# l13039968960/stm32H7-YOLO

Measured on AMD Instinct MI355X. Metric: images/sec int8 YOLO-face 56x56, higher is better.
Workload: dtype int8; 1 GPU; BASELINE configs[1]: batch=4096 int8 YOLO-face 56x56x3 frames per GPU, fused LDS-resident forward + GPU box decode; frames_per_gpu=4096, global_batch=4096, frame_bytes_in=9408, frame_bytes_out=882, input_batches_rotated=8, input_bytes_resident=308281344, kernel=yoloface56_fused<F=2,NW=8>, requant_rounding=ref, parallelism=single GPU, gather_every=1, collectives_issued=0, launch_streams=2

## Files before the change

stm32h7-yolo_amd/csrc/yf_decode.hip.h:

```cpp
#ifndef YF_DECODE_HIP_H
#define YF_DECODE_HIP_H
#include <hip/hip_runtime.h>
#include <stdint.h>
#include "../../include/yf_network.h"

namespace yfdec {

__device__ __constant__ uint32_t d_sig_bits[256];
__device__ __constant__ uint32_t d_exp_bits[256];

__device__ __forceinline__ int f2i_x86(float v) {
  return (v > -2147483904.0f && v < 2147483648.0f) ? (int)v : (int)0x80000000;
}
__device__ __forceinline__ int f2i_sat(float v) {
  return v != v ? 0 : (v >= 2147483648.0f ? 0x7FFFFFFF : (v <= -2147483648.0f ? (int)0x80000000 : (int)v));
}
__device__ __forceinline__ int dbl_wrap(int v) { return (int)((unsigned)v * 2u); }

__device__ __forceinline__ void decode_frame(const int8_t* head, long frame, int lane, int mode, float w_scale, float h_scale,
                                             yf_det* __restrict__ dets, int* __restrict__ counts, int cap) {
  yf_det* out = dets + frame * cap;
  const float anc_w[3] = {9.f, 12.f, 22.f}, anc_h[3] = {14.f, 17.f, 21.f};
  int total = 0;
  for (int base = 0; base < 147; base += 64) {
    const int i = base + lane;
    bool keep = false;
    int a = 0, row = 0, col = 0;
    const int8_t* p = head;
    float conf = 0.f;
    if (i < 147) {
      if (mode == YF_DECODE_PY) { a = i / 49; const int cell = i - a * 49; row = cell / 7; col = cell - row * 7; }
      else { const int cell = i / 3; a = i - cell * 3; row = cell / 7; col = cell - row * 7; }
      p = head + (row * 7 + col) * 18 + a * 6;
      conf = __uint_as_float(d_sig_bits[p[4] + 128]);
      keep = (mode == YF_DECODE_PY) ? (conf > 0.7f) : ((double)conf >= 0.7);
    }
    const unsigned long long mask = __ballot(keep);
    const int pos = total + __popcll(mask & ((1ull << lane) - 1ull));
    if (keep && pos < cap) {
      const float sx = __uint_as_float(d_sig_bits[p[0] + 128]), sy = __uint_as_float(d_sig_bits[p[1] + 128]);
      const float ew = __uint_as_float(d_exp_bits[p[2] + 128]), eh = __uint_as_float(d_exp_bits[p[3] + 128]);
      yf_det d;
      d.frame = (int32_t)frame; d.anchor = (uint8_t)a; d.row = (uint8_t)row; d.col = (uint8_t)col;
      d.q_conf = p[4]; d.conf = conf;
      const float cx = (sx + (float)col) * 8.f, cy = (sy + (float)row) * 8.f;
      const float bw = ew * anc_w[a], bh = eh * anc_h[a];
      if (mode == YF_DECODE_PY) {
        float x1 = cx - bw / 2, y1 = cy - bh / 2, x2 = cx + bw / 2, y2 = cy + bh / 2;
        x1 *= w_scale; x2 *= w_scale; y1 *= h_scale; y2 *= h_scale;
        d.x1 = f2i_x86(x1); d.y1 = f2i_x86(y1); d.x2 = f2i_x86(x2); d.y2 = f2i_x86(y2);
      } else {
        const float fy2 = cx - bw / 2, fy1 = cx + bw / 2, fx1 = cy - bh / 2, fx2 = cy + bh / 2;
        const bool arm = mode == YF_DECODE_FW;
        int y2 = arm ? f2i_sat(fy2) : f2i_x86(fy2), y1 = arm ? f2i_sat(fy1) : f2i_x86(fy1);
        int x1 = arm ? f2i_sat(fx1) : f2i_x86(fx1), x2 = arm ? f2i_sat(fx2) : f2i_x86(fx2);
        if (x1 < 0) x1 = 0;
        if (y1 < 0) y1 = 0;
        if (x2 > 55) x2 = 55;
        if (y2 > 55) y2 = 55;
        d.x1 = dbl_wrap(x1); d.y1 = dbl_wrap(y1); d.x2 = dbl_wrap(x2); d.y2 = dbl_wrap(y2);
      }
      out[pos] = d;
    }
    total += __popcll(mask);
  }
  if (lane == 0) counts[frame] = total;
}

typedef const __attribute__((address_space(3))) uint32_t* dec_lds_u32;
__device__ __forceinline__ void decode_frame_lds(const int8_t* head, long frame, int lane, int mode, float w_scale, float h_scale,
                                                 yf_det* __restrict__ dets, int* __restrict__ counts, int cap, uint32_t lds_tabs, int q_thr) {
  yf_det* out = dets + frame * cap;
  const float anc_w[3] = {9.f, 12.f, 22.f}, anc_h[3] = {14.f, 17.f, 21.f};
  auto sig = [&](int q) { return __uint_as_float(*(dec_lds_u32)(lds_tabs + 4u * (uint32_t)(q + 128))); };
  auto ex = [&](int q) { return __uint_as_float(*(dec_lds_u32)(lds_tabs + 1024u + 4u * (uint32_t)(q + 128))); };
  int pos[3], off[3], q4[3];
  bool keep[3];
  int total = 0;
#pragma unroll
  for (int c = 0; c < 3; ++c) {
    const int i = min(64 * c + lane, 146);
    if (mode == YF_DECODE_PY) { const int a = (i >= 49) + (i >= 98); off[c] = (i - 49 * a) * 18 + 6 * a; }
    else off[c] = 6 * i;
    q4[c] = head[off[c] + 4];
  }
#pragma unroll
  for (int c = 0; c < 3; ++c) {
    keep[c] = (64 * c + lane < 147) && q4[c] >= q_thr;
    const unsigned long long mask = __ballot(keep[c]);
    pos[c] = total + __popcll(mask & ((1ull << lane) - 1ull));
    total += __popcll(mask);
  }
#pragma unroll
  for (int c = 0; c < 3; ++c) {
    if (keep[c] && pos[c] < cap) {
      const int i = 64 * c + lane;
      int a, row, col;
      if (mode == YF_DECODE_PY) { a = i / 49; const int cell = i - a * 49; row = cell / 7; col = cell - row * 7; }
      else { const int cell = i / 3; a = i - cell * 3; row = cell / 7; col = cell - row * 7; }
      const int8_t* q = head + off[c];
      const float sx = sig(q[0]), sy = sig(q[1]), ew = ex(q[2]), eh = ex(q[3]);
      yf_det d;
      d.frame = (int32_t)frame; d.anchor = (uint8_t)a; d.row = (uint8_t)row; d.col = (uint8_t)col;
      d.q_conf = (int8_t)q4[c]; d.conf = sig(q4[c]);
      const float cx = (sx + (float)col) * 8.f, cy = (sy + (float)row) * 8.f;
      const float bw = ew * anc_w[a], bh = eh * anc_h[a];
      if (mode == YF_DECODE_PY) {
        float x1 = cx - bw / 2, y1 = cy - bh / 2, x2 = cx + bw / 2, y2 = cy + bh / 2;
        x1 *= w_scale; x2 *= w_scale; y1 *= h_scale; y2 *= h_scale;
        d.x1 = f2i_x86(x1); d.y1 = f2i_x86(y1); d.x2 = f2i_x86(x2); d.y2 = f2i_x86(y2);
      } else {
        const float fy2 = cx - bw / 2, fy1 = cx + bw / 2, fx1 = cy - bh / 2, fx2 = cy + bh / 2;
        const bool arm = mode == YF_DECODE_FW;
        int y2 = arm ? f2i_sat(fy2) : f2i_x86(fy2), y1 = arm ? f2i_sat(fy1) : f2i_x86(fy1);
        int x1 = arm ? f2i_sat(fx1) : f2i_x86(fx1), x2 = arm ? f2i_sat(fx2) : f2i_x86(fx2);
        if (x1 < 0) x1 = 0;
        if (y1 < 0) y1 = 0;
        if (x2 > 55) x2 = 55;
        if (y2 > 55) y2 = 55;
        d.x1 = dbl_wrap(x1); d.y1 = dbl_wrap(y1); d.x2 = dbl_wrap(x2); d.y2 = dbl_wrap(y2);
      }
      out[pos[c]] = d;
    }
  }
  if (lane == 0) counts[frame] = total;
}

}
#endif
```

stm32h7-yolo_amd/csrc/yf_engine.hip:

```cpp
#include <hip/hip_runtime.h>
#include <stdio.h>
#include <stdlib.h>
#include <string.h>
#include <condition_variable>
#include <deque>
#include <mutex>
#include <string>
#include <thread>
#include "yf_engine.h"
#include "yf_stream_scratch.h"
#include "yf_decode.hip.h"
#define YF_SET
#include "yf_kernel_set.hip.h"
#define YF_SET u
#define YF_RQ3_DENSE 1
#include "yf_kernel_set.hip.h"
#define YF_SET x
#define YF_RQ_FP32 1
#include "yf_kernel_set.hip.h"
#ifdef YF_LAB
#define YF_DUMP_PROD_ORDER 1
#define YF_SET
#include "yf_kernel_set.hip.h"
#define YF_SET u
#define YF_RQ3_DENSE 1
#include "yf_kernel_set.hip.h"
#undef YF_DUMP_PROD_ORDER
#endif
#include "gen/yf_decode_tables_gen.h"

namespace {

using yfdec::d_sig_bits;
using yfdec::d_exp_bits;

__global__ void __launch_bounds__(256) decode_kernel(const int8_t* __restrict__ heads, long n, int mode, float w_scale,
                                                     float h_scale, yf_det* __restrict__ dets, int* __restrict__ counts, int cap) {
  const int lane = threadIdx.x & 63;
  const long frame = (long)blockIdx.x * 4 + (threadIdx.x >> 6);
  if (frame >= n) return;
  yfdec::decode_frame(heads + frame * 882, frame, lane, mode, w_scale, h_scale, dets, counts, cap);
}

__global__ void __launch_bounds__(256) pack_dets_kernel(const yf_det* __restrict__ dets, const int* __restrict__ counts, const int8_t* __restrict__ heads,
                                                        uint32_t* __restrict__ wire, long n, int cap) {
  const long i = (long)blockIdx.x * 256 + threadIdx.x;
  if (i >= n * cap) return;
  const long f = i / cap;
  const int k = (int)(i - f * cap);
  uint32_t w0 = 0, w1 = 0, w2 = 0;
  if (k < min(counts[f], cap)) {
    const yf_det d = dets[i];
    const int8_t* q = heads + f * 882 + ((int)d.row * 7 + (int)d.col) * 18 + 6 * (int)d.anchor;
    w0 = (uint32_t)d.anchor | ((uint32_t)d.row << 8) | ((uint32_t)d.col << 16);
    w1 = (uint32_t)(uint8_t)q[0] | ((uint32_t)(uint8_t)q[1] << 8) | ((uint32_t)(uint8_t)q[2] << 16) | ((uint32_t)(uint8_t)q[3] << 24);
    w2 = (uint32_t)(uint8_t)q[4] | ((uint32_t)(uint8_t)q[5] << 8);
  }
  wire[3 * i] = w0; wire[3 * i + 1] = w1; wire[3 * i + 2] = w2;
}
__global__ void __launch_bounds__(256) unpack_dets_kernel(const uint32_t* __restrict__ wire, const int* __restrict__ counts, int8_t* __restrict__ heads, long n, int cap) {
  const int lane = threadIdx.x & 63;
  const long f = (long)blockIdx.x * 4 + (threadIdx.x >> 6);
  if (f >= n) return;
  int8_t* h = heads + f * 882;
  for (int b = lane; b < 882; b += 64) h[b] = (int8_t)-128;
  __builtin_amdgcn_wave_barrier();
  __threadfence_block();
  const int m = min(counts[f], cap);
  for (int k = lane; k < m; k += 64) {
    const uint32_t w0 = wire[3 * (f * cap + k)], w1 = wire[3 * (f * cap + k) + 1], w2 = wire[3 * (f * cap + k) + 2];
    const int a = (int)(w0 & 255u), row = (int)((w0 >> 8) & 255u), col = (int)((w0 >> 16) & 255u);
    if (a > 2 || row > 6 || col > 6) continue;
    int8_t* q = h + (row * 7 + col) * 18 + 6 * a;
    q[0] = (int8_t)(w1 & 255u); q[1] = (int8_t)((w1 >> 8) & 255u); q[2] = (int8_t)((w1 >> 16) & 255u); q[3] = (int8_t)(w1 >> 24);
    q[4] = (int8_t)(w2 & 255u); q[5] = (int8_t)((w2 >> 8) & 255u);
  }
}

__global__ void __launch_bounds__(256) prepare_rgb565_kernel(const uint8_t* __restrict__ src, int8_t* __restrict__ dst, long n) {
  const long i = (long)blockIdx.x * 256 + threadIdx.x;
  if (i >= n * 3136) return;
  const long f = i / 3136; const int r = (int)(i - f * 3136);
  const int y = r / 56, x = r - y * 56;
  const uint8_t* s = src + f * (112 * 112 * 2);
  unsigned sr = 0, sg = 0, sb = 0;
#pragma unroll
  for (int dy = 0; dy < 2; ++dy)
#pragma unroll
    for (int dx = 0; dx < 2; ++dx) {
      const int o = ((2 * y + dy) * 112 + (2 * x + dx)) * 2;
      const unsigned px = ((unsigned)s[o] << 8) | s[o + 1];
      sr += (px >> 11) & 0x1F; sg += (px >> 5) & 0x3F; sb += px & 0x1F;
    }
  const unsigned color = (((sr >> 2) & 0x1F) << 11) | (((sg >> 2) & 0x3F) << 5) | ((sb >> 2) & 0x1F);
  int8_t* o8 = dst + f * 9408 + r * 3;
  o8[0] = (int8_t)(((color & 0xF800) >> 8) - 128);
  o8[1] = (int8_t)(((color & 0x07E0) >> 3) - 128);
  o8[2] = (int8_t)(((color & 0x001F) << 3) - 128);
}

typedef void (*fused_fn)(const yf::NetParams);
enum Build { RUN, DUMP, DUMP_PROD_ORDER, CAMERA };
struct Variant { int f, nw, kset; Build build; fused_fn fn; size_t lds; size_t park; const char* name; };

#define YF_KERNEL_SETS(X) \
  X( , 0, "", "") \
  X(u, 1, ",sign-free dense epilogue", " (sign-free dense epilogue)") \
  X(x, 2, ",fp32 requantisation", " (fp32 requantisation)")
#define YF_VARIANT(NS, KSET, F, NW, BUILD, TAG) { F, NW, KSET, BUILD, (fused_fn)NS::yoloface56_fused<F, NW, BUILD == DUMP || BUILD == DUMP_PROD_ORDER, BUILD == CAMERA>, \
    NS::lds_bytes<F, NW, BUILD == DUMP || BUILD == DUMP_PROD_ORDER>(), NS::scratch_bytes_per_frame_slot<BUILD == DUMP || BUILD == DUMP_PROD_ORDER>(), \
    "yoloface56_fused<F=" #F ",NW=" #NW TAG ">" },
#define YF_PRODUCT_VARIANTS(S, KSET, LABEL, BAND_LABEL) \
  YF_VARIANT(yf##S, KSET, 2, 8, RUN, LABEL) YF_VARIANT(yf##S, KSET, 1, 8, RUN, LABEL) YF_VARIANT(yf##S, KSET, 2, 8, DUMP, LABEL) \
  YF_VARIANT(yf##S, KSET, 2, 8, CAMERA, ",RGB565 input" LABEL)
const Variant k_variants[] = {
  YF_KERNEL_SETS(YF_PRODUCT_VARIANTS)
#ifdef YF_LAB
  YF_VARIANT(yf, 0, 1, 4, RUN, "") YF_VARIANT(yf, 0, 2, 4, RUN, "") YF_VARIANT(yf, 0, 4, 8, RUN, "") YF_VARIANT(yf, 0, 2, 4, DUMP, "")
  YF_VARIANT(yfpd, 0, 2, 8, DUMP_PROD_ORDER, ",dump in production order")
  YF_VARIANT(yfpdu, 1, 2, 8, DUMP_PROD_ORDER, ",dump in production order,sign-free dense epilogue")
#endif
};

}

struct yf_engine {
  int device = 0;
  int cus = 0;
  size_t lds_per_cu = 0;
  int band_wgs_per_cu[3][3] = {{1, 1, 1}, {1, 1, 1}, {1, 1, 1}};
  int kset = 0;
#ifdef YF_LAB
  int grid_div = 1;
  int fail_next_launch = 0;
  bool dump_prod_order = false;
#endif
  uint8_t* d_tab = nullptr;
  yf_table_index ix;
  const Variant* var = nullptr;
  const Variant* var_dump = nullptr;
  void* d_in = nullptr; void* d_out = nullptr; long stage_cap = 0;
  bool layerwise160 = false;
  long chunk160 = 1024;
  yf_stream_scratch arena160;
  yf_stream_scratch park; size_t park_region = 0;
  hipStream_t own_stream = nullptr;
  hipEvent_t ev0 = nullptr, ev1 = nullptr;
  std::string err;
  uint32_t sig_bits[256], exp_bits[256];
  const Variant* var_small = nullptr;
  hipStream_t pipe_stream[2] = {nullptr, nullptr};
  hipEvent_t pipe_ev[2] = {nullptr, nullptr};
  void* h_small_in = nullptr; void* h_small_out = nullptr;
  struct Downloader* dl = nullptr;
};
constexpr long SMALL_N = 512;
constexpr long ZERO_COPY_N = 8;
constexpr long PIPE_MIN_N = 2048, PIPE_CHUNK_DEFAULT = 3072, PIPE_LAST_DEFAULT = 1024;

struct Downloader {
  struct Job { hipEvent_t ready; const void* src; void* dst; size_t bytes; };
  int device = 0;
  hipStream_t stream = nullptr;
  std::thread th;
  std::mutex mu;
  std::condition_variable cv_job, cv_idle;
  std::deque<Job> q;
  int pending = 0;
  bool stop = false;
  hipError_t status = hipSuccess;
  void loop() {
    (void)hipSetDevice(device);
    for (;;) {
      Job j;
      {
        std::unique_lock<std::mutex> lk(mu);
        cv_job.wait(lk, [&] { return stop || !q.empty(); });
        if (q.empty()) return;
        j = q.front(); q.pop_front();
      }
      hipError_t rc = hipStreamWaitEvent(stream, j.ready, 0);
      if (rc == hipSuccess) rc = hipMemcpyAsync(j.dst, j.src, j.bytes, hipMemcpyDeviceToHost, stream);
      if (rc == hipSuccess) rc = hipStreamSynchronize(stream);
      {
        std::lock_guard<std::mutex> lk(mu);
        if (rc != hipSuccess && status == hipSuccess) status = rc;
        --pending; cv_idle.notify_all();
      }
    }
  }
  hipError_t start(int dev) {
    device = dev;
    const hipError_t rc = hipStreamCreateWithFlags(&stream, hipStreamNonBlocking);
    if (rc != hipSuccess) return rc;
    th = std::thread([this] { loop(); });
    return hipSuccess;
  }
  void submit(const Job& j) { { std::lock_guard<std::mutex> lk(mu); q.push_back(j); ++pending; } cv_job.notify_one(); }
  hipError_t drain() { std::unique_lock<std::mutex> lk(mu); cv_idle.wait(lk, [&] { return pending == 0; }); const hipError_t rc = status; status = hipSuccess; return rc; }
  hipError_t drain_to(int below) { std::unique_lock<std::mutex> lk(mu); cv_idle.wait(lk, [&] { return pending < below; }); return status; }
  ~Downloader() {
    { std::lock_guard<std::mutex> lk(mu); stop = true; }
    cv_job.notify_all();
    if (th.joinable()) th.join();
    if (stream) (void)hipStreamDestroy(stream);
  }
};

#define HIPCHK(e_, call) do { hipError_t rc_ = (call); if (rc_ != hipSuccess) { \
    (e_)->err = std::string(#call) + ": " + hipGetErrorString(rc_); return YF_ENG_ERR_HIP; } } while (0)

static const Variant* shape_for(const yf_engine* e, long n);
static const Variant* find_variant(int f, int nw, int kset, Build build) {
  for (const Variant& v : k_variants) if (v.f == f && v.nw == nw && v.kset == kset && v.build == build) return &v;
  return nullptr;
}

static const Variant* dump_variant_for(const yf_engine* e, int f, int nw) {
#ifdef YF_LAB
  if (e->dump_prod_order) {
    const Variant* v = find_variant(f, nw, e->kset, DUMP_PROD_ORDER);
    if (v || e->kset == 2) return v;
  }
#endif
  return find_variant(f, nw, e->kset, DUMP);
}
static void select_variants(yf_engine* e, int f, int nw, bool automatic) {
  e->var = find_variant(f, nw, e->kset, RUN);
  e->var_dump = dump_variant_for(e, f, nw);
  e->var_small = automatic ? find_variant(1, 8, e->kset, RUN) : nullptr;
}

#ifdef YF_LAB
template <int ST>
static int launch160_from(yf_engine* e, const yf160::GenParams& prm, unsigned grid, hipStream_t s) {
  if constexpr (ST < yf160::GEN_STAGES) {
    hipLaunchKernelGGL((yf160::generic_stage_kernel<ST, 8>), dim3(grid), dim3(512), yf160::LUT_BYTES, s, prm);
    { hipError_t rc_ = hipGetLastError(); if (rc_ != hipSuccess) { e->err = std::string("generic stage launch: ") + hipGetErrorString(rc_); return YF_ENG_ERR_HIP; } }
    return launch160_from<ST + 1>(e, prm, grid, s);
  } else {
    return YF_ENG_OK;
  }
}

#endif

struct BandKernel { const void* fn; const char* name; unsigned threads; size_t lds; int jobs_per_frame; };
#ifndef YF_K1_NW
#define YF_K1_NW 8
#endif
#define YF_K1_NW_ YF_K1_NW
#define YF_BAND_KERNELS(S, KSET, LABEL, BAND_LABEL) \
  {{(const void*)yf160##S::band::band_k1<YF_K1_NW_>, "band_k1" BAND_LABEL, YF_K1_NW_ * 64, (size_t)yf160##S::band::K1_LDS, yf160##S::band::K1_BANDS}, \
   {(const void*)yf160##S::band::band_k23<8>, "band_k23" BAND_LABEL, 512, (size_t)yf160##S::band::K23_LDS, yf160##S::band::K23_BANDS}, \
   {(const void*)yf160##S::band::band_k4<8>,  "band_k4" BAND_LABEL, 512,  (size_t)yf160##S::band::K4_LDS, 1}},
static const BandKernel k_band_fused[3][3] = { YF_KERNEL_SETS(YF_BAND_KERNELS) };
static int launch160_banded(yf_engine* e, const yf160::band::Params& prm, hipStream_t s) {
  for (int i = 0; i < 3; ++i) {
    const BandKernel& k = k_band_fused[e->kset][i];
    const long jobs = prm.n * k.jobs_per_frame;
    const long full = (long)e->cus * e->band_wgs_per_cu[e->kset][i];
    const unsigned grid = (unsigned)(jobs < full ? jobs : full);
    void* args[] = {(void*)&prm};
    const hipError_t rc = hipLaunchKernel(k.fn, dim3(grid), dim3(k.threads), args, k.lds, s);
    if (rc != hipSuccess) { e->err = std::string(k.name) + " launch: " + hipGetErrorString(rc); return YF_ENG_ERR_HIP; }
  }
  return YF_ENG_OK;
}

static const char k_layout_refusal[] = "table blob layout differs from the layout compiled into the kernels";
static bool layout_is_the_compiled_plan(const yf_table_index* ix) {
  bool same = (int)ix->lut_off == yf::PLAN.lut_off && (int)ix->total_bytes == yf::PLAN.total;
  for (int i = 0; i < YF_N_DENSE; ++i) same = same && (int)ix->dense[i].w_off == yf::PLAN.w_off[i] && (int)ix->dense[i].c_off == yf::PLAN.c_off[i];
  for (int i = 0; i < YF_N_DW; ++i) same = same && (int)ix->dw[i].g_off == yf::PLAN.g_off[i];
  for (int i = 0; i < YF_N_CS; ++i)
    same = same && (int)ix->cs_v_off[i] == yf::PLAN.vb_off[i] && (int)ix->cs_v_bytes[i] == yf::PLAN.vb_bytes[i] && (int)ix->cs_s_off[i] == yf::PLAN.sb_off[i];
  return same;
}

template <typename Kernel, typename... Args>
static int launch_small(yf_engine* e, Kernel kernel, long threads, void* stream, Args... args) {
  if (threads == 0) return YF_ENG_OK;
  HIPCHK(e, hipSetDevice(e->device));
  hipLaunchKernelGGL(kernel, dim3((unsigned)((threads + 255) / 256)), dim3(256), 0, (hipStream_t)stream, args...);
  HIPCHK(e, hipGetLastError());
  return YF_ENG_OK;
}

static int upload_decode_tables(yf_engine* e, const uint32_t* sig, const uint32_t* ex) {
  for (int i = 1; i < 256; ++i) {
    float a, b; memcpy(&a, &sig[i - 1], 4); memcpy(&b, &sig[i], 4);
    if (!(b >= a)) { e->err = "sigmoid table is not monotonic"; return YF_ENG_ERR_ARG; }
  }
  HIPCHK(e, hipSetDevice(e->device));
  HIPCHK(e, hipDeviceSynchronize());
  HIPCHK(e, hipMemcpyToSymbol(HIP_SYMBOL(d_sig_bits), sig, 1024));
  HIPCHK(e, hipMemcpyToSymbol(HIP_SYMBOL(d_exp_bits), ex, 1024));
  memcpy(e->sig_bits, sig, 1024); memcpy(e->exp_bits, ex, 1024);
  return YF_ENG_OK;
}

extern "C" {

int yf_engine_set_decode_tables(yf_engine* e, const uint32_t* sig_bits, const uint32_t* exp_bits) {
  if (!e || !sig_bits || !exp_bits) return YF_ENG_ERR_ARG;
  return upload_decode_tables(e, sig_bits, exp_bits);
}
void yf_engine_get_decode_tables(const yf_engine* e, uint32_t* sig_bits, uint32_t* exp_bits) {
  memcpy(sig_bits, e->sig_bits, 1024); memcpy(exp_bits, e->exp_bits, 1024);
}

int yf_engine_create(int device, const uint8_t* table_blob, const yf_table_index* ix, int kernel_set, yf_engine** out, char* err, size_t errlen) {
  auto fail = [&](const std::string& m, int code) { if (err && errlen) snprintf(err, errlen, "%s", m.c_str()); return code; };
  if (!table_blob || !ix || !out) return fail("bad arguments", YF_ENG_ERR_ARG);
  int ndev = 0;
  hipError_t rc = hipGetDeviceCount(&ndev);
  if (rc != hipSuccess || ndev <= 0)
    return fail(std::string("no HIP device: ") + (rc != hipSuccess ? hipGetErrorString(rc) : "device count is 0"), YF_ENG_ERR_NO_DEVICE);
  if (device < 0 || device >= ndev) return fail("device index out of range", YF_ENG_ERR_ARG);
  yf_engine* e = new yf_engine();
  e->device = device; e->ix = *ix;
  e->arena160.max_regions = 4;
  auto bail = [&](hipError_t r, const char* what) { std::string m = std::string(what) + ": " + hipGetErrorString(r); yf_engine_destroy(e); return fail(m, YF_ENG_ERR_HIP); };
  auto quit = [&](const std::string& m, int code) { yf_engine_destroy(e); return fail(m, code); };
  if ((rc = hipSetDevice(device)) != hipSuccess) return bail(rc, "hipSetDevice");
  hipDeviceProp_t prop;
  if ((rc = hipGetDeviceProperties(&prop, device)) != hipSuccess) return bail(rc, "hipGetDeviceProperties");
  if (strncmp(prop.gcnArchName, "gfx950", 6) != 0) return quit(std::string("unsupported GPU ") + prop.gcnArchName + " (this library is gfx950 only)", YF_ENG_ERR_NO_DEVICE);
  e->cus = prop.multiProcessorCount;
  e->lds_per_cu = prop.maxSharedMemoryPerMultiProcessor;
  for (const Variant& v : k_variants)
    if (e->lds_per_cu < v.lds) return quit("the device reports " + std::to_string(e->lds_per_cu) + " bytes of LDS per CU, " + v.name + " needs " + std::to_string(v.lds), YF_ENG_ERR_NO_DEVICE);
  if (!layout_is_the_compiled_plan(ix)) return quit(k_layout_refusal, YF_ENG_ERR_ARG);
  if ((rc = hipMalloc((void**)&e->d_tab, ix->total_bytes)) != hipSuccess) return bail(rc, "hipMalloc(tables)");
  if ((rc = hipMemcpy(e->d_tab, table_blob, ix->total_bytes, hipMemcpyHostToDevice)) != hipSuccess) return bail(rc, "hipMemcpy(tables)");
  if (upload_decode_tables(e, yf_sigmoid_bits, yf_exp_bits) != YF_ENG_OK) { const std::string m = e->err; return quit(m, YF_ENG_ERR_HIP); }
  auto prepare_kernel = [&](const void* fn, const std::string& refusal, size_t lds, unsigned threads = 0, int* wgs_per_cu = nullptr) -> int {
    hipFuncAttributes at;
    if ((rc = hipFuncGetAttributes(&at, fn)) != hipSuccess) return bail(rc, "hipFuncGetAttributes");
    if (at.sharedSizeBytes != 0) return quit(refusal, YF_ENG_ERR_HIP);
    if (lds && (rc = hipFuncSetAttribute(fn, hipFuncAttributeMaxDynamicSharedMemorySize, (int)lds)) != hipSuccess) return bail(rc, "hipFuncSetAttribute(max dynamic LDS)");
    if (!wgs_per_cu) return YF_ENG_OK;
    int occ = 0;
    if ((rc = hipOccupancyMaxActiveBlocksPerMultiprocessor(&occ, fn, (int)threads, lds)) != hipSuccess) return bail(rc, "hipOccupancyMaxActiveBlocksPerMultiprocessor");
    *wgs_per_cu = occ > 0 ? occ : 1;
    return YF_ENG_OK;
  };
  const std::string static_lds = ": kernel has static LDS, absolute LUT addressing is invalid";
  int r;
  for (const Variant& v : k_variants) if ((r = prepare_kernel((const void*)v.fn, v.name + static_lds, v.lds)) != YF_ENG_OK) return r;
#ifdef YF_LAB
  if ((r = prepare_kernel((const void*)yf160::generic_stage_kernel<1, 8>, "generic stage kernel has static LDS", 0)) != YF_ENG_OK) return r;
  { const char* lw = getenv("YF_160_LAYERWISE"); e->layerwise160 = lw && lw[0] == '1'; }
#endif
  for (int u = 0; u < 3; ++u)
    for (int i = 0; i < 3; ++i) {
      const BandKernel& k = k_band_fused[u][i];
      if ((r = prepare_kernel(k.fn, k.name + static_lds, k.lds, k.threads, &e->band_wgs_per_cu[u][i])) != YF_ENG_OK) return r;
    }
  { const char* ck = getenv("YF_160_CHUNK"); if (ck && atol(ck) > 0) e->chunk160 = atol(ck); }
#ifdef YF_LAB
  { const char* fl = getenv("YF_LAB_FAIL_LAUNCHES"); if (fl) e->fail_next_launch = atoi(fl); }
  { const char* gd = getenv("YF_LAB_GRID_DIV"); if (gd && atoi(gd) > 1) e->grid_div = atoi(gd); }
  { const char* pd = getenv("YF_LAB_DUMP_PROD_ORDER"); e->dump_prod_order = pd && pd[0] == '1'; }
#endif
  {
    size_t park = 0;
    for (const Variant& v : k_variants) park = v.park > park ? v.park : park;
    size_t slots = 4;
    for (const Variant& v : k_variants) { const size_t need = (e->lds_per_cu / v.lds) * (size_t)v.f; slots = need > slots ? need : slots; }
    e->park_region = (size_t)e->cus * slots * park;
  }
  if ((rc = hipStreamCreate(&e->own_stream)) != hipSuccess) return bail(rc, "hipStreamCreate");
  if ((rc = hipEventCreate(&e->ev0)) != hipSuccess || (rc = hipEventCreate(&e->ev1)) != hipSuccess) return bail(rc, "hipEventCreate");
  for (int k = 0; k < 2; ++k) {
    if ((rc = hipStreamCreateWithFlags(&e->pipe_stream[k], hipStreamNonBlocking)) != hipSuccess) return bail(rc, "hipStreamCreateWithFlags");
    if ((rc = hipEventCreateWithFlags(&e->pipe_ev[k], hipEventDisableTiming)) != hipSuccess) return bail(rc, "hipEventCreateWithFlags");
  }
  if ((rc = hipHostMalloc(&e->h_small_in, (size_t)ZERO_COPY_N * 9408, hipHostMallocMapped)) != hipSuccess ||
      (rc = hipHostMalloc(&e->h_small_out, (size_t)ZERO_COPY_N * 882, hipHostMallocMapped)) != hipSuccess) return bail(rc, "hipHostMalloc(pinned staging)");
  e->kset = kernel_set;
  select_variants(e, 2, 8, true);
  *out = e;
  return YF_ENG_OK;
}

int yf_engine_set_tables(yf_engine* e, const uint8_t* table_blob, const yf_table_index* ix, int kernel_set) {
  if (!e || !table_blob || !ix) return YF_ENG_ERR_ARG;
  if (!find_variant(e->var->f, e->var->nw, kernel_set, RUN)) { e->err = "the configured kernel shape has no build for this rounding"; return YF_ENG_ERR_VARIANT; }
  if (!layout_is_the_compiled_plan(ix)) { e->err = k_layout_refusal; return YF_ENG_ERR_ARG; }
  HIPCHK(e, hipSetDevice(e->device));
  HIPCHK(e, hipDeviceSynchronize());
  HIPCHK(e, hipMemcpy(e->d_tab, table_blob, ix->total_bytes, hipMemcpyHostToDevice));
  e->ix = *ix;
  const bool automatic = e->var_small != nullptr;
  e->kset = kernel_set;
  select_variants(e, e->var->f, e->var->nw, automatic);
  return YF_ENG_OK;
}

void yf_engine_destroy(yf_engine* e) {
  if (!e) return;
  (void)hipSetDevice(e->device);
  (void)hipDeviceSynchronize();
  if (e->d_tab) (void)hipFree(e->d_tab);
  if (e->d_in) (void)hipFree(e->d_in);
  if (e->d_out) (void)hipFree(e->d_out);
  e->arena160.release();
  e->park.release();
  if (e->ev0) (void)hipEventDestroy(e->ev0);
  if (e->ev1) (void)hipEventDestroy(e->ev1);
  if (e->own_stream) (void)hipStreamDestroy(e->own_stream);
  delete e->dl;
  for (int k = 0; k < 2; ++k) {
    if (e->pipe_ev[k]) (void)hipEventDestroy(e->pipe_ev[k]);
    if (e->pipe_stream[k]) (void)hipStreamDestroy(e->pipe_stream[k]);
  }
  if (e->h_small_in) (void)hipHostFree(e->h_small_in);
  if (e->h_small_out) (void)hipHostFree(e->h_small_out);
  delete e;
}

int yf_engine_table_plan(int32_t* out, int cap) {
  const int need = 2 * YF_N_DENSE + YF_N_DW + 2 + 3 * YF_N_CS;
  if (!out || cap < need) return need;
  int k = 0;
  for (int i = 0; i < YF_N_DENSE; ++i) out[k++] = yf::PLAN.w_off[i];
  for (int i = 0; i < YF_N_DENSE; ++i) out[k++] = yf::PLAN.c_off[i];
  for (int i = 0; i < YF_N_DW; ++i) out[k++] = yf::PLAN.g_off[i];
  out[k++] = yf::PLAN.lut_off; out[k++] = yf::PLAN.total;
  for (int i = 0; i < YF_N_CS; ++i) out[k++] = yf::PLAN.vb_off[i];
  for (int i = 0; i < YF_N_CS; ++i) out[k++] = yf::PLAN.vb_bytes[i];
  for (int i = 0; i < YF_N_CS; ++i) out[k++] = yf::PLAN.sb_off[i];
  return need;
}

int yf_engine_variant_exists(int frames_per_wg, int waves_per_wg) { return find_variant(frames_per_wg, waves_per_wg, 0, RUN) != nullptr; }

int yf_engine_configure(yf_engine* e, int frames_per_wg, int waves_per_wg) {
  if (!e) return YF_ENG_ERR_ARG;
  if (frames_per_wg < 0) {
    select_variants(e, 2, 8, true);
    return YF_ENG_OK;
  }
  const int f = frames_per_wg > 0 ? frames_per_wg : e->var->f, nw = waves_per_wg > 0 ? waves_per_wg : e->var->nw;
  if (!find_variant(f, nw, e->kset, RUN)) { e->err = "no such kernel variant"; return YF_ENG_ERR_VARIANT; }
  select_variants(e, f, nw, false);
  return YF_ENG_OK;
}

const char* yf_engine_error(const yf_engine* e) { return e ? e->err.c_str() : "null engine"; }
const char* yf_engine_kernel_name(const yf_engine* e) { return e && e->var ? e->var->name : ""; }
const char* yf_engine_kernel_name_for(const yf_engine* e, long n) { return e && e->var ? shape_for(e, n)->name : ""; }
#ifndef YF_BUILD_ID
#define YF_BUILD_ID "unstamped"
#endif
const char* yf_engine_build_id(void) { return YF_BUILD_ID; }
long yf_engine_dump_bytes(void) { return yf::DumpOffsets::TOTAL; }

static int yf_decode_q_threshold(const yf_engine* e, int mode) {
  for (int i = 0; i < 256; ++i) {
    float v; memcpy(&v, &e->sig_bits[i], 4);
    if (mode == YF_DECODE_PY ? (v > 0.7f) : ((double)v >= 0.7)) return i - 128;
  }
  return 128;
}
static bool decode_mode_ok(int mode) { return mode == YF_DECODE_PY || mode == YF_DECODE_FW || mode == YF_DECODE_FW_HOST; }
struct DecodeArgs { void* dets; void* counts; int cap, mode; float w_scale, h_scale; };

static const Variant* shape_for(const yf_engine* e, long n) { return (e->var_small && n <= SMALL_N) ? e->var_small : e->var; }

static int launch(yf_engine* e, const Variant* v, const void* d_in, void* d_out, void* d_dump, long n, hipStream_t s, int stop_stage = -1,
                  const DecodeArgs* dec = nullptr) {
  if (n <= 0) return YF_ENG_OK;
  if (((uintptr_t)d_in & 3) != 0) { e->err = "input must be 4-byte aligned"; return YF_ENG_ERR_ARG; }
  if (((uintptr_t)d_out & 1) != 0) { e->err = "output must be 2-byte aligned"; return YF_ENG_ERR_ARG; }
  yf::NetParams prm;
  prm.in = (const int8_t*)d_in; prm.out = (int8_t*)d_out; prm.n = n; prm.tab = e->d_tab; prm.dump = (int8_t*)d_dump; prm.stop_stage = stop_stage;
  prm.dets = nullptr; prm.counts = nullptr; prm.cap = 0; prm.mode = 0; prm.w_scale = prm.h_scale = 1.f;
  prm.q_thr = 128;
  if (dec) { prm.dets = (yf_det*)dec->dets; prm.counts = (int*)dec->counts; prm.cap = dec->cap; prm.mode = dec->mode; prm.w_scale = dec->w_scale; prm.h_scale = dec->h_scale;
             prm.q_thr = yf_decode_q_threshold(e, dec->mode); }
  const long groups = (n + v->f - 1) / v->f;
  const int per_cu = (int)(e->lds_per_cu / v->lds) > 0 ? (int)(e->lds_per_cu / v->lds) : 1;
  long grid = (long)e->cus * per_cu;
#ifdef YF_LAB
  if (e->grid_div > 1) grid = grid / e->grid_div > 0 ? grid / e->grid_div : 1;
#endif
  if (grid > groups) grid = groups;
  prm.scratch = nullptr;
  yf_stream_scratch::Lease lease;
  if (v->park) {
    const size_t need = (size_t)grid * v->f * v->park;
    if (need > e->park_region) { e->err = "tail scratch region too small for this kernel shape"; return YF_ENG_ERR_VARIANT; }
    HIPCHK(e, e->park.get(s, e->park_region, &lease));
    prm.scratch = lease.ptr;
  }
#ifdef YF_LAB
  if (e->fail_next_launch > 0) { --e->fail_next_launch; grid = 0; }
#endif
  hipLaunchKernelGGL(v->fn, dim3((unsigned)grid), dim3(v->nw * 64), v->lds, s, prm);
  HIPCHK(e, hipGetLastError());
  HIPCHK(e, lease.mark());
  return YF_ENG_OK;
}

int yf_engine_run_device(yf_engine* e, const void* d_in, void* d_out, void* d_dump, long n, void* stream) {
  if (!e || !d_in || !d_out || n < 0) return YF_ENG_ERR_ARG;
  HIPCHK(e, hipSetDevice(e->device));
#ifdef YF_BARPROF
  return launch(e, e->var, d_in, d_out, d_dump, n, (hipStream_t)stream);
#else
  if (d_dump && !e->var_dump) { e->err = "no debug (dump) build of the configured kernel shape"; return YF_ENG_ERR_VARIANT; }
  return launch(e, d_dump ? e->var_dump : shape_for(e, n), d_in, d_out, d_dump, n, (hipStream_t)stream);
#endif
}

int yf_engine_run_decode_device(yf_engine* e, const void* d_in, void* d_out, long n, int mode, float w_scale, float h_scale,
                                void* d_dets, void* d_counts, int cap, void* stream) {
  if (!e || !d_in || !d_out || !d_dets || !d_counts || n < 0 || cap <= 0 || !decode_mode_ok(mode)) return YF_ENG_ERR_ARG;
  HIPCHK(e, hipSetDevice(e->device));
  const DecodeArgs dec = {d_dets, d_counts, cap, mode, w_scale, h_scale};
  return launch(e, shape_for(e, n), d_in, d_out, nullptr, n, (hipStream_t)stream, -1, &dec);
}

int yf_engine_run_camera_device(yf_engine* e, const void* d_rgb565, void* d_out, long n, int mode, float w_scale, float h_scale,
                                void* d_dets, void* d_counts, int cap, void* stream) {
  if (!e || !d_rgb565 || !d_out || n < 0) return YF_ENG_ERR_ARG;
  if (d_dets && (!d_counts || cap <= 0 || !decode_mode_ok(mode))) return YF_ENG_ERR_ARG;
  if (((uintptr_t)d_rgb565 & 15) != 0) { e->err = "camera frames must be 16-byte aligned"; return YF_ENG_ERR_ARG; }
  HIPCHK(e, hipSetDevice(e->device));
  const Variant* v = find_variant(e->var->f, e->var->nw, e->kset, CAMERA);
  if (!v) { e->err = "no camera-input build of the configured kernel shape"; return YF_ENG_ERR_VARIANT; }
  const DecodeArgs dec = {d_dets, d_counts, cap, mode, w_scale, h_scale};
  return launch(e, v, d_rgb565, d_out, nullptr, n, (hipStream_t)stream, -1, d_dets ? &dec : nullptr);
}

int yf_engine_run_host(yf_engine* e, const void* h_in, void* h_out, long n) {
  if (!e || !h_in || n < 0) return YF_ENG_ERR_ARG;
  if (n == 0) return YF_ENG_OK;
  HIPCHK(e, hipSetDevice(e->device));
  if (n <= ZERO_COPY_N) {
    memcpy(e->h_small_in, h_in, (size_t)n * 9408);
    void *d_i = nullptr, *d_o = nullptr;
    HIPCHK(e, hipHostGetDevicePointer(&d_i, e->h_small_in, 0));
    HIPCHK(e, hipHostGetDevicePointer(&d_o, e->h_small_out, 0));
    const int rc = launch(e, shape_for(e, n), d_i, d_o, nullptr, n, e->own_stream);
    if (rc) return rc;
    HIPCHK(e, hipStreamSynchronize(e->own_stream));
    if (h_out) memcpy(h_out, e->h_small_out, (size_t)n * 882);
    return YF_ENG_OK;
  }
  if (n > e->stage_cap) {
    if (e->d_in) (void)hipFree(e->d_in);
    if (e->d_out) (void)hipFree(e->d_out);
    e->d_in = e->d_out = nullptr; e->stage_cap = 0;
    HIPCHK(e, hipMalloc(&e->d_in, (size_t)n * 9408));
    HIPCHK(e, hipMalloc(&e->d_out, (size_t)n * 882));
    e->stage_cap = n;
  }
  if (n < PIPE_MIN_N) {
    HIPCHK(e, hipMemcpyAsync(e->d_in, h_in, (size_t)n * 9408, hipMemcpyHostToDevice, e->own_stream));
    const int rc = launch(e, shape_for(e, n), e->d_in, e->d_out, nullptr, n, e->own_stream);
    if (rc) return rc;
    if (h_out) HIPCHK(e, hipMemcpyAsync(h_out, e->d_out, (size_t)n * 882, hipMemcpyDeviceToHost, e->own_stream));
    HIPCHK(e, hipStreamSynchronize(e->own_stream));
    return YF_ENG_OK;
  }
  if (h_out && !e->dl) {
    e->dl = new Downloader();
    const hipError_t rc = e->dl->start(e->device);
    if (rc != hipSuccess) { delete e->dl; e->dl = nullptr; e->err = std::string("download stream: ") + hipGetErrorString(rc); return YF_ENG_ERR_HIP; }
  }
  static const long PIPE_CHUNK = [] { const char* v = getenv("YF_PIPE_CHUNK"); const long c = v ? atol(v) : 0; return c >= 256 ? c : PIPE_CHUNK_DEFAULT; }();
  static const long PIPE_LAST = [] { const char* v = getenv("YF_PIPE_LAST"); const long c = v ? atol(v) : 0; return c >= 64 ? c : PIPE_LAST_DEFAULT; }();
  int rc = YF_ENG_OK;
  hipError_t hrc = hipSuccess;
  long done = 0;
  for (int k = 0; done < n && rc == YF_ENG_OK && hrc == hipSuccess; ++k) {
    long c = n - done < PIPE_CHUNK ? n - done : PIPE_CHUNK;
    if (c == n - done && c > 2 * PIPE_LAST) c -= PIPE_LAST;
    hipStream_t st = e->pipe_stream[k & 1];
    const char* src = (const char*)h_in + done * 9408;
    char* d_i = (char*)e->d_in + done * 9408;
    char* d_o = (char*)e->d_out + done * 882;
    if (h_out && k >= 2) { const hipError_t r = e->dl->drain_to(2); if (r != hipSuccess) { hrc = r; break; } }
    hrc = hipMemcpyAsync(d_i, src, (size_t)c * 9408, hipMemcpyHostToDevice, st);
    if (hrc != hipSuccess) break;
    rc = launch(e, e->var, d_i, d_o, nullptr, c, st);
    if (rc != YF_ENG_OK) break;
    if (h_out) {
      hrc = hipEventRecord(e->pipe_ev[k & 1], st);
      if (hrc != hipSuccess) break;
      e->dl->submit(Downloader::Job{e->pipe_ev[k & 1], d_o, (char*)h_out + done * 882, (size_t)c * 882});
    }
    done += c;
  }
  const hipError_t d_rc = e->dl && h_out ? e->dl->drain() : hipSuccess;
  const hipError_t s0 = hipStreamSynchronize(e->pipe_stream[0]), s1 = hipStreamSynchronize(e->pipe_stream[1]);
  if (rc != YF_ENG_OK) return rc;
  for (hipError_t r : {hrc, d_rc, s0, s1}) if (r != hipSuccess) { e->err = std::string("pipelined host run: ") + hipGetErrorString(r); return YF_ENG_ERR_HIP; }
  return YF_ENG_OK;
}

int yf_engine_run_host_dump(yf_engine* e, const void* h_in, void* h_out, void* h_dump, long n) {
  if (!e || !h_in || !h_out || !h_dump || n <= 0) return YF_ENG_ERR_ARG;
  if (!e->var_dump) { e->err = "no debug (dump) build of the configured kernel shape"; return YF_ENG_ERR_VARIANT; }
  HIPCHK(e, hipSetDevice(e->device));
  const size_t ds = (size_t)yf::DumpOffsets::TOTAL;
  char *d_i = nullptr, *d_o = nullptr, *d_d = nullptr;
  int rc = YF_ENG_OK;
  hipError_t h = hipMalloc((void**)&d_i, (size_t)n * 9408);
  if (h == hipSuccess) h = hipMalloc((void**)&d_o, (size_t)n * 882);
  if (h == hipSuccess) h = hipMalloc((void**)&d_d, (size_t)n * ds);
  if (h == hipSuccess) h = hipMemcpyAsync(d_i, h_in, (size_t)n * 9408, hipMemcpyHostToDevice, e->own_stream);
  if (h == hipSuccess) rc = launch(e, e->var_dump, d_i, d_o, d_d, n, e->own_stream);
  if (h == hipSuccess && rc == YF_ENG_OK) h = hipMemcpyAsync(h_out, d_o, (size_t)n * 882, hipMemcpyDeviceToHost, e->own_stream);
  if (h == hipSuccess && rc == YF_ENG_OK) h = hipMemcpyAsync(h_dump, d_d, (size_t)n * ds, hipMemcpyDeviceToHost, e->own_stream);
  const hipError_t hs = hipStreamSynchronize(e->own_stream);
  if (d_i) (void)hipFree(d_i);
  if (d_o) (void)hipFree(d_o);
  if (d_d) (void)hipFree(d_d);
  if (rc != YF_ENG_OK) return rc;
  if (h != hipSuccess || hs != hipSuccess) { e->err = std::string("observed run: ") + hipGetErrorString(h != hipSuccess ? h : hs); return YF_ENG_ERR_HIP; }
  return YF_ENG_OK;
}

long yf_engine_dump_offset(int tflite_op) {
  typedef yf::DumpOffsets D;
  switch (tflite_op) {
    case 2: return D::T1; case 4: return D::T2; case 5: return D::T3; case 7: return D::T4; case 21: return D::Q21; case 11: return D::T6;
    case 12: return D::T7; case 14: return D::T8; case 16: return D::T9; case 18: return D::T11; case 22: return D::T14; case 24: return D::T15;
    case 45: return D::Q45; case 28: return D::T17; case 29: return D::T18; case 31: return D::T19; case 33: return D::T20; case 35: return D::T22;
    case 37: return D::T23; case 39: return D::T24; case 41: return D::T26; case 46: return D::T30; case 48: return D::T31; case 50: return D::T32;
    case 52: return D::T33; case 8: return D::P8; case 17: return D::C17; case 25: return D::P25; case 34: return D::C34; case 40: return D::C40;
    case 43: return D::L43;
    default: return -1;
  }
}

static int time_launches(yf_engine* e, const Variant* v, const void* d_in, void* d_out, long n, int iters, int stop_stage, void* stream, float* ms_per_launch) {
  HIPCHK(e, hipSetDevice(e->device));
  hipStream_t s = (hipStream_t)stream;
  HIPCHK(e, hipEventRecord(e->ev0, s));
  for (int i = 0; i < iters; ++i) { const int rc = launch(e, v, d_in, d_out, nullptr, n, s, stop_stage); if (rc) return rc; }
  HIPCHK(e, hipEventRecord(e->ev1, s));
  HIPCHK(e, hipEventSynchronize(e->ev1));
  float ms = 0.f;
  HIPCHK(e, hipEventElapsedTime(&ms, e->ev0, e->ev1));
  *ms_per_launch = ms / iters;
  return YF_ENG_OK;
}

int yf_engine_time_device(yf_engine* e, const void* d_in, void* d_out, long n, int iters, void* stream, float* ms_per_launch) {
  if (!e || !d_in || !d_out || n <= 0 || iters <= 0 || !ms_per_launch) return YF_ENG_ERR_ARG;
  return time_launches(e, e->var, d_in, d_out, n, iters, -1, stream, ms_per_launch);
}

int yf_engine_time_stages(yf_engine* e, const void* d_in, void* d_out, long n, int iters, int stop_stage, void* stream, float* ms_per_launch) {
  if (!e || !d_in || !d_out || n <= 0 || iters <= 0 || !ms_per_launch) return YF_ENG_ERR_ARG;
  if (!e->var_dump) { e->err = "no debug (stage-timing) build of the configured kernel shape"; return YF_ENG_ERR_VARIANT; }
  return time_launches(e, e->var_dump, d_in, d_out, n, iters, stop_stage, stream, ms_per_launch);
}

int yf_engine_run_device_160(yf_engine* e, const void* d_in, void* d_out, long n, void* stream) {
  if (!e || !d_in || !d_out || n < 0) return YF_ENG_ERR_ARG;
  if (n == 0) return YF_ENG_OK;
  if (((uintptr_t)d_in & 3) != 0 || ((uintptr_t)d_out & 1) != 0) { e->err = "input must be 4-byte, output 2-byte aligned"; return YF_ENG_ERR_ARG; }
  HIPCHK(e, hipSetDevice(e->device));
  const long cap = n < e->chunk160 ? n : e->chunk160;
#ifdef YF_LAB
  const size_t per_frame = e->layerwise160 ? (size_t)yf160::FRAME_BYTES : (size_t)yf160::band::ARENA_BYTES;
#else
  const size_t per_frame = (size_t)yf160::band::ARENA_BYTES;
#endif
  yf_stream_scratch::Lease lease;
  HIPCHK(e, e->arena160.get((hipStream_t)stream, (size_t)cap * per_frame, &lease));
  char* arena = lease.ptr;
  for (long done = 0; done < n; done += cap) {
    const long m = (n - done) < cap ? (n - done) : cap;
    int rc;
#ifdef YF_LAB
    if (e->layerwise160) {
      if (e->kset == 2) { e->err = "the layer-by-layer 160x160 form has no float32-requantisation build (YF_160_LAYERWISE with YF_ROUND_FP32)"; return YF_ENG_ERR_VARIANT; }
      yf160::GenParams prm;
      prm.in = (const int8_t*)d_in + done * yf160::IN_FRAME_BYTES;
      prm.out = (int8_t*)d_out + done * yf160::OUT_FRAME_BYTES;
      prm.n = m; prm.tab = e->d_tab; prm.arena = arena;
      rc = launch160_from<0>(e, prm, (unsigned)m, (hipStream_t)stream);
    } else
#endif
    {
      yf160::band::Params prm;
      prm.in = (const int8_t*)d_in + done * yf160::IN_FRAME_BYTES;
      prm.out = (int8_t*)d_out + done * yf160::OUT_FRAME_BYTES;
      prm.n = m; prm.tab = e->d_tab; prm.arena = arena;
      rc = launch160_banded(e, prm, (hipStream_t)stream);
    }
    if (rc) return rc;
  }
  HIPCHK(e, lease.mark());
  return YF_ENG_OK;
}

int yf_engine_release_stream(yf_engine* e, void* stream) {
  if (!e) return YF_ENG_ERR_ARG;
  HIPCHK(e, hipSetDevice(e->device));
  HIPCHK(e, e->park.release_stream((hipStream_t)stream));
  HIPCHK(e, e->arena160.release_stream((hipStream_t)stream));
  return YF_ENG_OK;
}

size_t yf_engine_scratch_bytes(yf_engine* e) { return e ? e->park.bytes_held() + e->arena160.bytes_held() : 0; }
void yf_engine_scratch_stats(yf_engine* e, unsigned long long out[6]) {
  for (int i = 0; i < 6; ++i) out[i] = 0;
  if (!e) return;
  for (yf_stream_scratch* m : {&e->park, &e->arena160}) {
    const yf_stream_scratch::Stats s = m->stats();
    out[0] += s.events_recorded; out[1] += s.events_skipped; out[2] += s.event_waits; out[3] += s.device_syncs; out[4] += s.acquire_waits; out[5] += s.regions;
  }
}

int yf_engine_decode_device(yf_engine* e, const void* d_heads, long n, int mode, float w_scale, float h_scale,
                            void* d_dets, void* d_counts, int cap, void* stream) {
  if (!e || !d_heads || !d_dets || !d_counts || n < 0 || cap <= 0 || !decode_mode_ok(mode)) return YF_ENG_ERR_ARG;
  return launch_small(e, decode_kernel, n * 64, stream, (const int8_t*)d_heads, n, mode, w_scale, h_scale, (yf_det*)d_dets, (int*)d_counts, cap);
}

int yf_engine_pack_detections_device(yf_engine* e, const void* d_dets, const void* d_counts, const void* d_heads, void* d_wire, long n, int cap, void* stream) {
  if (!e || !d_dets || !d_counts || !d_heads || !d_wire || n < 0 || cap <= 0 || ((uintptr_t)d_wire & 3) != 0 || ((uintptr_t)d_dets & 3) != 0) return YF_ENG_ERR_ARG;
  return launch_small(e, pack_dets_kernel, n * cap, stream, (const yf_det*)d_dets, (const int*)d_counts, (const int8_t*)d_heads, (uint32_t*)d_wire, n, cap);
}

int yf_engine_unpack_detections_device(yf_engine* e, const void* d_wire, const void* d_counts, void* d_heads, long n, int cap, void* stream) {
  if (!e || !d_wire || !d_counts || !d_heads || n < 0 || cap <= 0 || ((uintptr_t)d_wire & 3) != 0) return YF_ENG_ERR_ARG;
  return launch_small(e, unpack_dets_kernel, n * 64, stream, (const uint32_t*)d_wire, (const int*)d_counts, (int8_t*)d_heads, n, cap);
}

int yf_engine_prepare_rgb565_device(yf_engine* e, const void* d_rgb565, void* d_out, long n, void* stream) {
  if (!e || !d_rgb565 || !d_out || n < 0) return YF_ENG_ERR_ARG;
  return launch_small(e, prepare_rgb565_kernel, n * 3136, stream, (const uint8_t*)d_rgb565, (int8_t*)d_out, n);
}

}
```

stm32h7-yolo_amd/csrc/yf_fused56.hip.h:

```cpp


template <class B, int C, int F, int NT>
__device__ __forceinline__ void dump_buf(const char* frames, int8_t* dump, long stride, long off, long first_frame,
                                         long n_frames, int tid, int ch0 = 0, int split = 1 << 30, int gap = 0) {
  if (!dump) return;
  for (int i = tid; i < F * B::P * C; i += NT) {
    const int ch = i % C; const int t = i / C;
    const int p = t % B::P; const int f = t / B::P;
    if (first_frame + f >= n_frames) continue;
    const int phys = ch0 + ch + (ch >= split ? gap : 0);
    dump[(first_frame + f) * stride + off + (long)p * C + ch] = (int8_t)frames[f * B::FS + B::at_p(p) + phys];
  }
}

template <class B, int C, int FT, int NT, class IdOf>
__device__ __forceinline__ void dump_sets(const char* frames, int8_t* dump, long stride, long off, const IdOf& id_of, int tid, int ch0 = 0, int split = 1 << 30, int gap = 0) {
  for (int i = tid; i < FT * B::P * C; i += NT) {
    const int ch = i % C; const int t = i / C;
    const int p = t % B::P; const int f = t / B::P;
    const long id = id_of(f);
    if (id < 0) continue;
    const int phys = ch0 + ch + (ch >= split ? gap : 0);
    dump[id * stride + off + (long)p * C + ch] = (int8_t)frames[f * B::FS + B::at_p(p) + phys];
  }
}

struct DumpOffsets {
  enum { T1 = 0, T2 = T1 + 6272, T3 = T2 + 6272, T4 = T3 + 3136, Q21 = T4 + 14112, T6 = Q21 + 3528, T7 = T6 + 3528,
         T8 = T7 + 1176, T9 = T8 + 7056, T11 = T9 + 7056, T14 = T11 + 1176, T15 = T14 + 7056, Q45 = T15 + 4704,
         T17 = Q45 + 1176, T18 = T17 + 1176, T19 = T18 + 392, T20 = T19 + 1960, T22 = T20 + 1960, T23 = T22 + 392,
         T24 = T23 + 1960, T26 = T24 + 1960, T30 = T26 + 392, T31 = T30 + 2352, T32 = T31 + 1960, T33 = T32 + 1960,
         P8 = T33 + 1568, C17 = P8 + 3528, P25 = C17 + 1176, C34 = P25 + 1176, C40 = C34 + 392, L43 = C40 + 392,
         TOTAL = L43 + 1176 };
};

struct NetParams {
  const int8_t* in;
  int8_t* out;
  long n;
  const uint8_t* tab;
  int8_t* dump;
  int stop_stage;
  yf_det* dets;
  int* counts;
  int cap, mode;
  int q_thr;
  float w_scale, h_scale;
  char* scratch;
};
static_assert(sizeof(yf_table_index) <= YF_INDEX_RESERVED, "index does not fit its reserved slot");

#ifndef YF_POOL_MERGE
#define YF_POOL_MERGE 1
#endif
#ifndef YF_POOL8H_WAVES
#define YF_POOL8H_WAVES 3
#endif
#ifndef YF_POOL8V_WAVES
#define YF_POOL8V_WAVES 3
#endif
#ifndef YF_PRIO_LIST
#define YF_PRIO_LIST 3,3,3,3,3,3,3,3,3,3, 2,2,2,2, 1,1,1,1,1,1, 0,0,0,0,0,0,0
#endif
constexpr int STAGE_PRIO[27] = {YF_PRIO_LIST};
template <int K> __device__ __forceinline__ void stage_prio() {
  if constexpr (K == 0 || STAGE_PRIO[K] != STAGE_PRIO[K - 1]) __builtin_amdgcn_s_setprio(STAGE_PRIO[K]);
}
#if defined(YF_LAB) && defined(YF_DUMP_PROD_ORDER)
#define YF_PDUMP 1
#else
#define YF_PDUMP 0
#endif
template <bool DUMP> constexpr bool tail_batch() { return !DUMP || YF_PDUMP; }

template <int F, int NW, bool DUMP, bool CAM = false>
#if !defined(YF_LAB) || !defined(YF_TPJ13)
#undef YF_TPJ13
#define YF_TPJ13 3
#endif
#if !defined(YF_LAB) || !defined(YF_TPJ23)
#undef YF_TPJ23
#define YF_TPJ23 2
#endif
#if defined(YF_LAB) && defined(YF_WHATIF_WPE)
#define YF_WPE(NW) YF_WHATIF_WPE
#else
#define YF_WPE(NW) ((NW) == 12 ? 6 : (NW) >= 8 ? 4 : ((NW) == 6 ? 3 : 2))
#endif
__global__ void __launch_bounds__(NW * 64, YF_WPE(NW)) yoloface56_fused(const NetParams prm) {
  extern __shared__ __attribute__((aligned(16))) char smem[];
  constexpr int NT = NW * 64;
  constexpr bool BATCH = tail_batch<DUMP>();
  constexpr bool POOL_MERGE = YF_POOL_MERGE != 0 && (!DUMP || YF_PDUMP) && NW >= 8;
  constexpr bool XDUMP = DUMP && !YF_PDUMP;
  typedef Buf<B_T14::OFF, 14, 14, 32, 14, 0, 0> B_T6X;
  typedef typename std::conditional<POOL_MERGE, B_T6X, B_T6>::type B_T6M;
  constexpr int FT = BATCH ? 2 * F : F;
  typedef TailBufs<BATCH ? FRAME_STRIDE / 2 : FRAME_STRIDE> U;
  constexpr int OUT_ALL_BYTES = BATCH ? 0 : (F * OUT_FRAME_BYTES + 15) & ~15;
  uint8_t* luts = reinterpret_cast<uint8_t*>(smem);
  constexpr int PRE = v2::pre_bytes<F, tail_batch<DUMP>()>();
  char* out_all = smem + PRE;
  char* frames = smem + PRE + OUT_ALL_BYTES;
  long parked_first = -1;
  const int tid0 = threadIdx.x;
  const uint8_t* __restrict__ tab = prm.tab;
  int vz = 0;
  asm volatile("" : "+v"(vz));
  for (int i = tid0; i < v2::LUT_B / 16; i += NT)
    reinterpret_cast<uint4*>(luts)[i] = reinterpret_cast<const uint4*>(tab + PLAN.lut_off)[i];
  for (int i = tid0; i < v2::ZERO_B / 16; i += NT) reinterpret_cast<uint4*>(smem + v2::ZERO)[i] = uint4{0, 0, 0, 0};
  constexpr int DBG_LUT = PRE + OUT_ALL_BYTES + FRAME_BYTES + (F - 1) * FRAME_STRIDE;
  if constexpr (DUMP) { if (tid0 < YF_DBG_LUT_BYTES / 16) reinterpret_cast<uint4*>(smem + DBG_LUT)[tid0] = reinterpret_cast<const uint4*>(tab + PLAN.lut_off + YF_N_LUT * 256 + YF_ADDLUT_BYTES)[tid0]; }
#if !(defined(YF_LAB) && defined(YF_WHATIF_NO_PROLOGUE_TABLES))
  {
    typedef v2::JobTabs<F, tail_batch<DUMP>()> JTS;
    typedef typename JTS::U UT;
    v2::fill_jobtab<F, 1, B_T1, B_T2, JTS::JT_DW3>(smem, tid0);
    v2::fill_jobtab<F, 2, B_T4, B_T6M, JTS::JT_DW10>(smem, tid0);
    v2::fill_jobtab<F, 1, B_T8, B_T9, JTS::JT_DW15>(smem, tid0);
    v2::fill_jobtab<JTS::FT, 2, typename UT::T15, typename UT::T17, JTS::JT_DW27>(smem, tid0);
    v2::fill_jobtab<JTS::FT, 1, typename UT::T19, typename UT::T20, JTS::JT_DW32>(smem, tid0);
    typedef v2::HaloTabs<F, tail_batch<DUMP>()> HTS;
    v2::build_halotab<typename HTS::G1, HTS::H_T1, NT>(smem, tid0);
    v2::build_halotab<typename HTS::G4, HTS::H_T4, NT>(smem, tid0);
    v2::build_halotab<typename HTS::G8, HTS::H_T8, NT>(smem, tid0);
    v2::build_halotab<typename HTS::G15, HTS::H_T15, NT>(smem, tid0);
    v2::build_halotab<typename HTS::G19, HTS::H_T19, NT>(smem, tid0);
  }
#endif

  const long n_groups = (prm.n + F - 1) / F;
  const AddK no_add = {};
  auto addctx = [&](int k) {
    const uint8_t* a = tab + offsetof(yf_table_index, add) + k * sizeof(yf_add);
    return AddK{uniform_u32(a + offsetof(yf_add, mo2)), uniform_u32(a + offsetof(yf_add, zro)),
                (unsigned long)uniform_u32(a + offsetof(yf_add, c64o)) | ((unsigned long)uniform_u32(a + offsetof(yf_add, c64o) + 4) << 32),
                (int)uniform_u32(a + offsetof(yf_add, rso))};
  };
  constexpr long DS = DumpOffsets::TOTAL;
#ifdef YF_BARPROF
  bool prof_on = false;
  int bar_no = 0;
  long long* prof_out = reinterpret_cast<long long*>(prm.dump) + ((long)blockIdx.x * NW + __builtin_amdgcn_readfirstlane(tid0 >> 6)) * 80;
#define YF_SYNC() do { asm volatile("s_waitcnt vmcnt(0)" ::: "memory");    \
                       if (prof_on && (tid0 & 63) == 0 && bar_no < 40) prof_out[2 * bar_no] = __builtin_readcyclecounter(); __syncthreads(); \
                       if (prof_on && (tid0 & 63) == 0 && bar_no < 40) prof_out[2 * bar_no + 1] = __builtin_readcyclecounter(); ++bar_no; } while (0)
#else
#define YF_SYNC() do { asm volatile("s_waitcnt vmcnt(0)" ::: "memory"); __syncthreads(); } while (0)
#endif
#define YF_HALO(B, RING, FR, G, HOFF, WI, TID) \
  v2::fill_halo_t<B, typename v2::HaloTabs<F, BATCH>::G, v2::HaloTabs<F, BATCH>::HOFF>(frames, load_halo_zp(tab, WI), TID)
#define YF_FETCH(CS, WV, LN) v2::fetch_consts<CS>(tab, WV, LN)
#define YF_CONV1(WV, LN, CS) v2::conv1_2_stage<F, NW, CS>(frames, tab, WV, LN)
#define YF_DENSE(FR, TPJ, KS, BW, IN, OUT, CH0, COUT, EPI, LUT, ADDB, DI, AD, WV, LN, CS) \
  v2::dense2_stage<FR, NW, TPJ, KS, BW, IN, OUT, CH0, COUT, EPI, LUT, ADDB, CS>(frames, out_all, tab, AD, WV, LN)
#define YF_DW(FR, STRIDE, IN, OUT, C, LUT, WI, WV, LN, CS, JTOFF) v2::dw2_stage<FR, NW, STRIDE, IN, OUT, C, LUT, CS, v2::JobTabs<F, BATCH>::JTOFF>(frames, tab, WV, LN)
#define YF_DUMP(BUF, C, OFF, ...) \
  if constexpr (DUMP) { if (prm.dump) { dump_buf<BUF, C, F, NT>(frames, prm.dump, DS, DumpOffsets::OFF, first, prm.n, tid, ##__VA_ARGS__); YF_SYNC(); } }
  int stage_no = 0;
#define YF_STAGE_END() if constexpr (DUMP) { if (++stage_no == prm.stop_stage) continue; }
#define YF_PRIO(K) stage_prio<K>()

  long prev_first = -1;
  auto decode_prev = [&](int w, int ln) {
    if (prm.dets != nullptr && prev_first >= 0 && w >= NW - F && prev_first + (w - (NW - F)) < prm.n) {
      int dl = ln;
      asm volatile("" : "+v"(dl));
      yfdec::decode_frame(reinterpret_cast<const int8_t*>(out_all) + (w - (NW - F)) * OUT_FRAME_BYTES, prev_first + (w - (NW - F)), dl,
                          prm.mode, prm.w_scale, prm.h_scale, prm.dets, prm.counts, prm.cap);
    }
  };
  for (long grp = blockIdx.x; grp < n_groups; grp += gridDim.x) {
    const long first = grp * F;
#ifdef YF_BARPROF
    bar_no = 0;
    prof_on = !DUMP && prm.dump != nullptr && grp == (long)blockIdx.x + gridDim.x;
#endif
    int tid = tid0, tid_f = tid0, tid_m = tid0, tid_t = tid0;
    if constexpr ((YF_LAUNDER & 1) != 0) asm volatile("" : "+v"(tid_f));
    if constexpr ((YF_LAUNDER & 2) != 0) asm volatile("" : "+v"(tid_m));
    if constexpr ((YF_LAUNDER & 4) != 0) asm volatile("" : "+v"(tid_t));
    const int lane = tid & 63;
    const int wave = __builtin_amdgcn_readfirstlane(tid >> 6);
    const int L_f = tid_f & 63, L_m = tid_m & 63, L_t = tid_t & 63;
    const int W_f = __builtin_amdgcn_readfirstlane(tid_f >> 6), W_m = __builtin_amdgcn_readfirstlane(tid_m >> 6), W_t = __builtin_amdgcn_readfirstlane(tid_t >> 6);
    (void)lane; (void)wave;
#if !defined(YF_BARPROF)
    asm volatile("s_waitcnt lgkmcnt(0)\n\ts_barrier" ::: "memory");
#else
    YF_SYNC();
#endif
    stage_no = 0;
    YF_PRIO(0);
    int tid_s = tid0;
    asm volatile("" : "+v"(tid_s));
    if constexpr (CAM) stage_input_cam<F, NT>(frames, reinterpret_cast<const uint8_t*>(prm.in), first, prm.n, (int)uniform_u32(tab + offsetof(yf_table_index, in_zp)), tid_s);
    else stage_input<F, NT>(frames, prm.in, first, prm.n, (int)uniform_u32(tab + offsetof(yf_table_index, in_zp)), tid_s);
    YF_FETCH(0, W_f, L_f);
    YF_HALO(B_T1, true, F, G1, H_T1, YF_W_DW3, tid_f);
    YF_SYNC();
    YF_STAGE_END()
    YF_PRIO(1);
    YF_FETCH(1, W_f, L_f);
    YF_CONV1(W_f, L_f, 0);
    YF_SYNC(); YF_DUMP(B_T1, 8, T1)
    YF_STAGE_END()
    YF_PRIO(2);
    YF_FETCH(2, W_f, L_f);
    YF_DW(F, 1, B_T1, B_T2, 8, YF_L_LEAKY4, YF_W_DW3, W_f, L_f, 1, JT_DW3);
    YF_SYNC(); YF_DUMP(B_T2, 8, T2)
    YF_STAGE_END()
    YF_PRIO(3);
    YF_FETCH(3, W_f, L_f);
    YF_DENSE(F, 1, 1, 8, B_T2, B_T3, 0, 4, EPI_RAW, 0, B_T3, YF_D_C5, no_add, W_f, L_f, 2);
    YF_SYNC(); YF_DUMP(B_T3, 4, T3)
    YF_STAGE_END()
    YF_PRIO(4);
    YF_HALO(B_T4, false, F, G4, H_T4, YF_W_DW10, tid_f);
    YF_FETCH(4, W_f, L_f);
    YF_DENSE(F, 5, 1, 4, B_T3, B_T4, 0, 18, EPI_LUT, YF_L_LEAKY7, B_T4, YF_D_C6, no_add, W_f, L_f, 3);
    YF_SYNC(); YF_DUMP(B_T4, 18, T4)
    YF_STAGE_END()
    if constexpr (POOL_MERGE) {
      constexpr int PH = YF_POOL8H_WAVES, PV = YF_POOL8V_WAVES;
      YF_PRIO(5);
      YF_FETCH(5, W_m, L_m);
      if (W_m < PH) pool8_h<F, PH * 64>(frames, tid_m);
      else v2::dw2_stage<F, NW - PH, 2, B_T4, B_T6M, 18, YF_L_LEAKY11, 4, v2::JobTabs<F, BATCH>::JT_DW10>(frames, tab, W_m - PH, L_m);
      YF_SYNC(); YF_DUMP(B_T6M, 18, T6)
      YF_PRIO(8);
      YF_FETCH(6, W_m, L_m);
      YF_DENSE(F, 1, 2, 16, B_T6M, B_T7, 0, 6, EPI_RAW, 0, B_T7, YF_D_C12, no_add, W_m, L_m, 5);
      YF_SYNC(); YF_DUMP(B_T7, 6, T7)
      YF_PRIO(9);
      YF_HALO(B_T8, true, F, G8, H_T8, YF_W_DW15, tid_m);
      YF_FETCH(7, W_m, L_m);
      if (W_m < PV) pool8_v<F, PV * 64, false>(frames, tid_m);
      else v2::dense2_stage<F, NW - PV, YF_TPJ13, 1, 8, B_T7, B_T8, 0, 36, EPI_LUT, YF_L_LEAKY14, B_T8, 6>(frames, out_all, tab, no_add, W_m - PV, L_m);
      YF_SYNC(); YF_DUMP(B_T14, 18, Q21) YF_DUMP(B_T8, 36, T8)
    } else {
  YF_PRIO(5);
#if !(defined(YF_LAB) && defined(YF_WHATIF_NO_POOL8H))
      pool8_h<F, NT>(frames, tid_f);
      YF_SYNC();
#endif
      YF_STAGE_END()
      YF_PRIO(6);
      pool8_v<F, NT, XDUMP>(frames, tid_m);
      YF_SYNC();
      YF_PRIO(7);
      YF_FETCH(5, W_m, L_m);
      YF_DW(F, 2, B_T4, B_T6, 18, YF_L_LEAKY11, YF_W_DW10, W_m, L_m, 4, JT_DW10);
      YF_SYNC(); YF_DUMP(B_T14, 18, Q21) YF_DUMP(B_T14, 18, P8, YF_T14_CONV_BASE) YF_DUMP(B_T6, 18, T6)
      YF_STAGE_END()
      YF_PRIO(8);
      YF_FETCH(6, W_m, L_m);
      YF_DENSE(F, 1, 2, 16, B_T6, B_T7, 0, 6, EPI_RAW, 0, B_T7, YF_D_C12, no_add, W_m, L_m, 5);
      YF_SYNC(); YF_DUMP(B_T7, 6, T7)
      YF_STAGE_END()
      YF_PRIO(9);
      YF_HALO(B_T8, true, F, G8, H_T8, YF_W_DW15, tid_m);
      YF_FETCH(7, W_m, L_m);
      YF_DENSE(F, YF_TPJ13, 1, 8, B_T7, B_T8, 0, 36, EPI_LUT, YF_L_LEAKY14, B_T8, YF_D_C13, no_add, W_m, L_m, 6);
      YF_SYNC(); YF_DUMP(B_T8, 36, T8)
      YF_STAGE_END()
    }
    YF_PRIO(10);
    YF_FETCH(8, W_m, L_m);
    YF_DW(F, 1, B_T8, B_T9, 36, YF_L_LEAKY16, YF_W_DW15, W_m, L_m, 7, JT_DW15);
    YF_SYNC(); YF_DUMP(B_T9, 36, T9)
    YF_STAGE_END()
    YF_PRIO(11);
    YF_FETCH(9, W_m, L_m);
    if constexpr (XDUMP)
      v2::dense2_stage<F, NW, 1, 3, 16, B_T9, B_T11, 0, 6, EPI_ADD, YF_A_ADD18, B_T7, 8, B_T14::OFF + YF_T14_CONV_BASE, B_T14::S>(frames, out_all, tab, addctx(YF_A_ADD18), W_m, L_m);
    else
    YF_DENSE(F, 1, 3, 16, B_T9, B_T11, 0, 6, EPI_ADD, YF_A_ADD18, B_T7, YF_D_C17, addctx(YF_A_ADD18), W_m, L_m, 8);
    YF_SYNC(); YF_DUMP(B_T11, 6, T11) if constexpr (XDUMP) { YF_DUMP(B_T14, 6, C17, YF_T14_CONV_BASE) }
    YF_STAGE_END()
    YF_PRIO(12);
    YF_FETCH(10, W_m, L_m);
    YF_DENSE(F, 3, 1, 8, B_T11, B_T14, YF_T14_CONV_BASE, 18, EPI_LUT, YF_L_LEAKY20, B_T14, YF_D_C19, no_add, W_m, L_m, 9);
    YF_SYNC(); YF_DUMP(B_T14, 36, T14, 0, 18, 2)
    YF_STAGE_END()
    YF_PRIO(13);
    if constexpr (BATCH) {
      if (parked_first >= 0) {
        constexpr int PV = TailBufs<FRAME_BYTES>::T15_BYTES / 16, WI = (PV + 63) / 64;
        const char* park = prm.scratch + (long)blockIdx.x * (F * PV * 16);
        for (int j = W_m; j < F * WI; j += NW) {
          const int f = j / WI, k0 = (j - f * WI) * 64;
          if (k0 + L_m < PV)
            __builtin_amdgcn_global_load_lds((const __attribute__((address_space(1))) void*)(uintptr_t)(park + (f * PV + k0 + L_m) * 16),
                                             (__attribute__((address_space(3))) void*)(uintptr_t)(uint32_t)(PRE + (2 * f + 1) * U::T15::FS + 16 * k0),
                                             16, 0, 0);
        }
      }
    }
    YF_HALO(B_T15, false, F, G15, H_T15, YF_W_DW27, tid_m);
    YF_FETCH(11, W_m, L_m);
    YF_DENSE(F, YF_TPJ23, 3, 16, B_T14, B_T15, 0, 24, EPI_LUT, YF_L_LEAKY24, B_T15, YF_D_C23, no_add, W_m, L_m, 10);
    if constexpr (BATCH) asm volatile("s_waitcnt vmcnt(0)" ::: "memory");
    YF_SYNC(); YF_DUMP(B_T15, 24, T15)
    YF_STAGE_END()
    long odd_first = -1;
    if constexpr (BATCH) {
      constexpr int V = U::T15_BYTES / 16;
      uint4* park = reinterpret_cast<uint4*>(prm.scratch) + (long)blockIdx.x * (F * V);
      if (parked_first < 0 && grp + gridDim.x < n_groups) {
        for (int i = tid_t; i < F * V; i += NT) {
          const int f = i / V, k = i - f * V;
          park[i] = *reinterpret_cast<const uint4*>(frames + f * FRAME_STRIDE + 16 * k);
        }
        parked_first = first;
        continue;
      }
      if (parked_first >= 0) {
        odd_first = parked_first;
        parked_first = -1;
      }
    }
    auto frame_of = [&](int f) -> long {
      long id = first + f;
      if constexpr (BATCH) id = (f & 1) ? (odd_first >= 0 ? odd_first + (f >> 1) : -1) : first + (f >> 1);
      return id < prm.n ? id : -1;
    };
#define YF_DUMP_T(BUF, C, OFF, ...) \
  if constexpr (DUMP) { if (prm.dump) { if constexpr (BATCH) dump_sets<BUF, C, FT, NT>(frames, prm.dump, DS, DumpOffsets::OFF, frame_of, tid, ##__VA_ARGS__); \
                                        else dump_buf<BUF, C, FT, NT>(frames, prm.dump, DS, DumpOffsets::OFF, first, prm.n, tid, ##__VA_ARGS__); \
                                        YF_SYNC(); } }
    YF_PRIO(14);
    YF_FETCH(12, W_t, L_t);
    {
      constexpr int PW = v2::pool25_waves<FT>();
      static_assert(PW < NW, "waves left for conv2d_27");
      if (W_t < PW) v2::pool25_cols<FT, typename U::T15, typename U::T30, XDUMP>(frames, W_t * 64 + L_t);
      else v2::dw2_stage<FT, NW - PW, 2, typename U::T15, typename U::T17, 24, YF_L_LEAKY28, 11, v2::JobTabs<F, BATCH>::JT_DW27>(frames, tab, W_t - PW, L_t);
    }
    YF_SYNC(); YF_DUMP_T(typename U::T30, 24, Q45) if constexpr (XDUMP) { YF_DUMP_T(typename U::T30, 24, P25, 24) } YF_DUMP_T(typename U::T17, 24, T17)
    YF_STAGE_END()
    YF_PRIO(15);
    YF_FETCH(13, W_t, L_t);
    YF_DENSE(FT, 1, 2, 16, typename U::T17, typename U::T18, 0, 8, EPI_RAW, 0, typename U::T18, YF_D_C29, no_add, W_t, L_t, 12);
    if constexpr (!BATCH) decode_prev(W_t, L_t);
    YF_SYNC(); YF_DUMP_T(typename U::T18, 8, T18)
    YF_STAGE_END()
    YF_PRIO(16);
    YF_HALO(typename U::T19, true, FT, G19, H_T19, YF_W_DW32, tid_t);
    YF_FETCH(14, W_t, L_t);
    YF_DENSE(FT, 5, 1, 8, typename U::T18, typename U::T19, 0, 40, EPI_LUT, YF_L_LEAKY31, typename U::T19, YF_D_C30, no_add, W_t, L_t, 13);
    YF_SYNC(); YF_DUMP_T(typename U::T19, 40, T19)
    YF_STAGE_END()
    YF_PRIO(17);
    YF_FETCH(15, W_t, L_t);
    YF_DW(FT, 1, typename U::T19, typename U::T20, 40, YF_L_LEAKY33, YF_W_DW32, W_t, L_t, 14, JT_DW32);
    YF_SYNC(); YF_DUMP_T(typename U::T20, 40, T20)
    YF_STAGE_END()
    YF_PRIO(18);
    YF_FETCH(16, W_t, L_t);
    if constexpr (XDUMP)
      v2::dense2_stage<FT, NW, 1, 3, 16, typename U::T20, typename U::T22, 0, 8, EPI_ADD, YF_A_ADD35, typename U::T18, 15, U::T30::OFF + 24, U::T30::S>(frames, out_all, tab, addctx(YF_A_ADD35), W_t, L_t);
    else
    YF_DENSE(FT, 1, 3, 16, typename U::T20, typename U::T22, 0, 8, EPI_ADD, YF_A_ADD35, typename U::T18, YF_D_C34, addctx(YF_A_ADD35), W_t, L_t, 15);
    YF_SYNC(); YF_DUMP_T(typename U::T22, 8, T22) if constexpr (XDUMP) { YF_DUMP_T(typename U::T30, 8, C34, 24) }
    YF_STAGE_END()
    YF_PRIO(19);
    YF_HALO(typename U::T19, true, FT, G19, H_T19, YF_W_DW38, tid_t);
    YF_FETCH(17, W_t, L_t);
    YF_DENSE(FT, 5, 1, 8, typename U::T22, typename U::T19, 0, 40, EPI_LUT, YF_L_LEAKY37, typename U::T19, YF_D_C36, no_add, W_t, L_t, 16);
    YF_SYNC(); YF_DUMP_T(typename U::T19, 40, T23)
    YF_STAGE_END()
    YF_PRIO(20);
    YF_FETCH(18, W_t, L_t);
    YF_DW(FT, 1, typename U::T19, typename U::T20, 40, YF_L_LEAKY39, YF_W_DW38, W_t, L_t, 17, JT_DW32);
    YF_SYNC(); YF_DUMP_T(typename U::T20, 40, T24)
    YF_STAGE_END()
    YF_PRIO(21);
    YF_FETCH(19, W_t, L_t);
    if constexpr (XDUMP)
      v2::dense2_stage<FT, NW, 1, 3, 16, typename U::T20, typename U::T26, 0, 8, EPI_ADD, YF_A_ADD41, typename U::T22, 18, U::T30::OFF + 24, U::T30::S>(frames, out_all, tab, addctx(YF_A_ADD41), W_t, L_t);
    else
    YF_DENSE(FT, 1, 3, 16, typename U::T20, typename U::T26, 0, 8, EPI_ADD, YF_A_ADD41, typename U::T22, YF_D_C40, addctx(YF_A_ADD41), W_t, L_t, 18);
    YF_SYNC(); YF_DUMP_T(typename U::T26, 8, T26) if constexpr (XDUMP) { YF_DUMP_T(typename U::T30, 8, C40, 24) }
    YF_STAGE_END()
    YF_PRIO(22);
    YF_FETCH(20, W_t, L_t);
    if constexpr (XDUMP)
      v2::dense2_stage<FT, NW, 2, 1, 8, typename U::T26, typename U::T30, 24, 24, EPI_LUT, YF_L_L43Q44, typename U::T30, 19, U::T20::OFF, U::T20::S, DBG_LUT>(frames, out_all, tab, no_add, W_t, L_t);
    else
    YF_DENSE(FT, 3, 1, 8, typename U::T26, typename U::T30, 24, 24, EPI_LUT, YF_L_L43Q44, typename U::T30, YF_D_C42, no_add, W_t, L_t, 19);
    YF_SYNC(); YF_DUMP_T(typename U::T30, 48, T30) if constexpr (XDUMP) { YF_DUMP_T(typename U::T20, 24, L43) }
    YF_STAGE_END()
    YF_PRIO(23);
    YF_HALO(typename U::T19, true, FT, G19, H_T19, YF_W_DW49, tid_t);
    YF_FETCH(21, W_t, L_t);
    YF_DENSE(FT, 2, 3, 16, typename U::T30, typename U::T19, 0, 40, EPI_LUT, YF_L_LEAKY48, typename U::T19, YF_D_C47, no_add, W_t, L_t, 20);
    YF_SYNC(); YF_DUMP_T(typename U::T19, 40, T31)
    YF_STAGE_END()
    YF_PRIO(24);
    YF_FETCH(22, W_t, L_t);
    YF_DW(FT, 1, typename U::T19, typename U::T20, 40, YF_L_LEAKY50, YF_W_DW49, W_t, L_t, 21, JT_DW32);
    YF_SYNC(); YF_DUMP_T(typename U::T20, 40, T32)
    YF_STAGE_END()
    YF_PRIO(25);
    YF_FETCH(23, W_t, L_t);
    if (BATCH && prm.dets != nullptr && W_t < 2) {
      int dl = L_t;
      asm volatile("" : "+v"(dl));
      const uint8_t* src = reinterpret_cast<const uint8_t*>(W_t == 0 ? yfdec::d_sig_bits : yfdec::d_exp_bits) + 16 * dl;
      const uint32_t dst = (uint32_t)(PRE + OUT_ALL_BYTES + 1024 * W_t);
      uint32_t keep;
      asm volatile("s_mov_b32 %0, m0\n\ts_mov_b32 m0, %2\n\ts_nop 0\n\tglobal_load_lds_dwordx4 %1, off\n\ts_mov_b32 m0, %0"
                   : "=&s"(keep) : "v"(src), "s"(dst) : "memory");
    }
    YF_DENSE(FT, 2, 3, 16, typename U::T20, typename U::T33, 0, 32, EPI_LUT, YF_L_LEAKY52, typename U::T33, YF_D_C51, no_add, W_t, L_t, 22);
    YF_SYNC(); YF_DUMP_T(typename U::T33, 32, T33)
    YF_STAGE_END()
    YF_PRIO(26);
    if constexpr (!BATCH) {
      YF_DENSE(FT, 1, 2, 16, typename U::T33, typename U::T33, 0, 18, EPI_HEAD, 0, typename U::T33, YF_D_C53, no_add, W_t, L_t, 23);
      YF_SYNC();
      const long valid = min((long)F, prm.n - first);
      const int n16 = (int)(valid * (OUT_FRAME_BYTES / 2));
      uint16_t* dst = reinterpret_cast<uint16_t*>(prm.out + first * OUT_FRAME_BYTES);
      const uint16_t* srcp = reinterpret_cast<const uint16_t*>(out_all);
      for (int i = tid; i < n16; i += NT) dst[i] = srcp[i];
      prev_first = first;
    } else {
      YF_DENSE(FT, 1, 2, 16, typename U::T33, typename U::HEAD, 0, 18, EPI_HEAD_LDS, 0, typename U::T33, YF_D_C53, no_add, W_t, L_t, 23);
      YF_SYNC();
      constexpr int H16 = OUT_FRAME_BYTES / 2;
      const bool split = prm.dets != nullptr && FT < NW;
      const int c0 = split ? tid_t - FT * 64 : tid_t, cstep = split ? NT - FT * 64 : NT;
      if (!split || W_t >= FT) {
        for (int i = c0; i < FT * H16; i += cstep) {
          const int f = i / H16, k = i - f * H16;
          const long id = frame_of(f);
          if (id >= 0) reinterpret_cast<uint16_t*>(prm.out + id * OUT_FRAME_BYTES)[k] = *reinterpret_cast<const uint16_t*>(frames + f * U::HEAD::FS + U::HEAD::OFF + 2 * k);
        }
      }
      for (int f = W_t; f < FT; f += NW) {
        const long id = frame_of(f);
        if (prm.dets != nullptr && id >= 0) {
          int dl = L_t;
          asm volatile("" : "+v"(dl));
          yfdec::decode_frame_lds(reinterpret_cast<const int8_t*>(frames + f * U::HEAD::FS + U::HEAD::OFF), id, dl, prm.mode, prm.w_scale, prm.h_scale, prm.dets, prm.counts, prm.cap,
                                  (uint32_t)(PRE + OUT_ALL_BYTES), prm.q_thr);
        }
      }
    }
#undef YF_DUMP_T
  }
  if constexpr (!BATCH) {
    const int tid = tid0, lane = tid & 63, wave = __builtin_amdgcn_readfirstlane(tid >> 6);
    decode_prev(wave, lane);
  }
#undef YF_HALO
#undef YF_FETCH
#undef YF_CONV1
#undef YF_DENSE
#undef YF_DW
#undef YF_DUMP
#undef YF_STAGE_END
#undef YF_PRIO
#undef YF_SYNC
}

template <int F, int NW, bool DUMP>
constexpr size_t lds_bytes() { return (size_t)v2::pre_bytes<F, tail_batch<DUMP>()>() + (tail_batch<DUMP>() ? 0 : (F * OUT_FRAME_BYTES + 15) & ~15) + (size_t)FRAME_BYTES + (size_t)(F - 1) * FRAME_STRIDE + (DUMP ? YF_DBG_LUT_BYTES : 0); }
template <bool DUMP>
constexpr size_t scratch_bytes_per_frame_slot() { return tail_batch<DUMP>() ? (size_t)TailBufs<FRAME_BYTES>::T15_BYTES : 0; }
#undef YF_PDUMP
```

stm32h7-yolo_amd/csrc/yf_kernels.hip.h:

```cpp
#include <hip/hip_runtime.h>
#include <stddef.h>
#include <stdint.h>
#include <type_traits>
#include "yf_tables.h"

#pragma clang diagnostic push
#pragma clang diagnostic ignored "-Wint-to-pointer-cast"
#if !defined(YF_LAB) || !defined(YF_LAUNDER)
#undef YF_LAUNDER
#define YF_LAUNDER 0
#endif
#define YF_ROW_SKEW 4
namespace YF_NS {

#ifndef YF_NOINLINE_STAGES
#define YF_STAGE_FN __device__ __forceinline__
#else
#define YF_STAGE_FN __device__ __attribute__((noinline))
#endif

typedef int v4i __attribute__((ext_vector_type(4)));
typedef short v2s __attribute__((ext_vector_type(2)));

#if !defined(YF_H0) || YF_H0 == 56
constexpr int FRAME_BYTES = 34176;
#endif
constexpr int LUT_BYTES = YF_N_LUT * 256 + YF_ADDLUT_BYTES;


#if !defined(YF_H0) || YF_H0 == 56
#if defined(YF_LAB) && defined(YF_WHATIF_FS)
constexpr int FRAME_STRIDE = YF_WHATIF_FS;
#else
constexpr int FRAME_STRIDE = FRAME_BYTES;
#endif
constexpr int BUF_FS = FRAME_STRIDE;
#else
constexpr int BUF_FS = 0;
#endif
template <int OFF_, int W_, int H_, int S_, int RS_, int PT_, int PL_, int FS_ = BUF_FS, int SK_ = 0>
struct Buf {
  static constexpr int OFF = OFF_, W = W_, H = H_, S = S_, RS = RS_, PT = PT_, PL = PL_, FS = FS_, SK = SK_;
  static constexpr int P = W_ * H_, ROWB = RS_ * S_ + SK_;
  __device__ static __forceinline__ int at(int y, int x) { return OFF_ + (y + PT_) * ROWB + (x + PL_) * S_; }
  __device__ static __forceinline__ int at_p(int p) {
    if constexpr (RS_ == W_ && PT_ == 0 && PL_ == 0) return OFF_ + p * S_;
    else { const int y = p / W_; return at(y, p - y * W_); }
  }
};

#ifndef YF_H0
#define YF_H0 56
#endif
constexpr int G0 = YF_H0, G1 = G0 / 2, G2 = G0 / 4, G3 = G0 / 8;
static_assert(G0 % 8 == 0 && G3 >= 4, "input size must be a multiple of 8 and at least 32");

#if YF_H0 == 56
typedef Buf<    0, 56, 56,  4, 60, 1, 4> B_IN;
typedef Buf<13696, 28, 28,  8, 30, 1, 1, BUF_FS, YF_ROW_SKEW> B_T1;
typedef Buf<21024, 28, 28,  8, 28, 0, 0> B_T2;
typedef Buf<16832, 28, 28,  4, 28, 0, 0> B_T3;
typedef Buf<    0, 28, 28, 20, 29, 1, 1> B_T4;
typedef Buf<16832, 14, 28, 20, 14, 0, 0> B_HB;
typedef Buf<24672, 14, 14, 48, 14, 0, 0> B_T14;
typedef Buf<16832, 14, 14, 32, 14, 0, 0> B_T6;
typedef Buf<    0, 14, 14,  8, 14, 0, 0> B_T7;
typedef Buf< 1568, 14, 14, 36, 16, 1, 1> B_T8;
typedef Buf<10784, 14, 14, 48, 14, 0, 0> B_T9;
typedef Buf<20192, 14, 14,  8, 14, 0, 0> B_T11;
typedef Buf<    0, 14, 14, 24, 15, 1, 1> B_T15;
typedef Buf< 5408,  7,  7, 48,  7, 0, 0> B_T30;
typedef Buf< 7760,  7,  7, 32,  7, 0, 0> B_T17;
typedef Buf< 9328,  7,  7,  8,  7, 0, 0> B_T18;
typedef Buf< 9728,  7,  7, 40,  9, 1, 1, BUF_FS, YF_ROW_SKEW> B_T19;
typedef Buf<13008,  7,  7, 48,  7, 0, 0> B_T20;
typedef Buf<15360,  7,  7,  8,  7, 0, 0> B_T22;
typedef Buf<15752,  7,  7,  8,  7, 0, 0> B_T26;
typedef Buf<16144,  7,  7, 32,  7, 0, 0> B_T33;
template <int FS_>
struct TailBufs {
  typedef Buf<    0, 14, 14, 24, 15, 1, 1, FS_> T15;
  typedef Buf< 5408,  7,  7, 48,  7, 0, 0, FS_> T30;
  typedef Buf< 7760,  7,  7, 32,  7, 0, 0, FS_> T17;
  typedef Buf< 9328,  7,  7,  8,  7, 0, 0, FS_> T18;
  typedef Buf< 9728,  7,  7, 40,  9, 1, 1, FS_, YF_ROW_SKEW> T19;
  typedef Buf<13008,  7,  7, 48,  7, 0, 0, FS_> T20;
  typedef Buf<15360,  7,  7,  8,  7, 0, 0, FS_> T22;
  typedef Buf<15752,  7,  7,  8,  7, 0, 0, FS_> T26;
  typedef Buf< 7760,  7,  7, 32,  7, 0, 0, FS_> T33;
  typedef Buf<16160,  7,  7, 18,  7, 0, 0, FS_> HEAD;
  static constexpr int END = 16160 + 882, T15_BYTES = 5408;
  static_assert(T19::OFF + 9 * T19::ROWB <= T20::OFF && T20::OFF + 49 * 48 <= T22::OFF && T26::OFF + 49 * 8 <= HEAD::OFF, "tail buffers do not overlap");
#if !(defined(YF_LAB) && defined(YF_WHATIF_FS))
  static_assert(END <= FS_, "a set fits its stride");
#endif
};
#else
constexpr int arena_next(int off, int bytes) { return (off + bytes + 64 + 63) & ~63; }
#define YF_SEQ(NAME, PREV_END, W_, H_, S_, RS_, PT_, PL_, ROWS_)                      \
  constexpr int NAME##_OFF = PREV_END;                                                \
  typedef Buf<NAME##_OFF, W_, H_, S_, RS_, PT_, PL_> NAME;                            \
  constexpr int NAME##_END = arena_next(NAME##_OFF, (ROWS_) * (RS_) * (S_));
YF_SEQ(B_IN,  0,         G0, G0,  4, G0 + 4, 1, 4, G0 + 1)
YF_SEQ(B_T1,  B_IN_END,  G1, G1,  8, G1 + 2, 1, 1, G1 + 2)
YF_SEQ(B_T2,  B_T1_END,  G1, G1,  8, G1,     0, 0, G1)
YF_SEQ(B_T3,  B_T2_END,  G1, G1,  4, G1,     0, 0, G1)
YF_SEQ(B_T4,  B_T3_END,  G1, G1, 20, G1 + 1, 1, 1, G1 + 1)
YF_SEQ(B_HB,  B_T4_END,  G2, G1, 20, G2,     0, 0, G1)
YF_SEQ(B_T14, B_HB_END,  G2, G2, 48, G2,     0, 0, G2)
YF_SEQ(B_T6,  B_T14_END, G2, G2, 32, G2,     0, 0, G2)
YF_SEQ(B_T7,  B_T6_END,  G2, G2,  8, G2,     0, 0, G2)
YF_SEQ(B_T8,  B_T7_END,  G2, G2, 36, G2 + 2, 1, 1, G2 + 2)
YF_SEQ(B_T9,  B_T8_END,  G2, G2, 48, G2,     0, 0, G2)
YF_SEQ(B_T11, B_T9_END,  G2, G2,  8, G2,     0, 0, G2)
YF_SEQ(B_T15, B_T11_END, G2, G2, 24, G2 + 1, 1, 1, G2 + 1)
YF_SEQ(B_T30, B_T15_END, G3, G3, 48, G3,     0, 0, G3)
YF_SEQ(B_T17, B_T30_END, G3, G3, 32, G3,     0, 0, G3)
YF_SEQ(B_T18, B_T17_END, G3, G3,  8, G3,     0, 0, G3)
YF_SEQ(B_T19, B_T18_END, G3, G3, 40, G3 + 2, 1, 1, G3 + 2)
YF_SEQ(B_T20, B_T19_END, G3, G3, 48, G3,     0, 0, G3)
YF_SEQ(B_T22, B_T20_END, G3, G3,  8, G3,     0, 0, G3)
YF_SEQ(B_T26, B_T22_END, G3, G3,  8, G3,     0, 0, G3)
YF_SEQ(B_T33, B_T26_END, G3, G3, 32, G3,     0, 0, G3)
#undef YF_SEQ
#endif

#if YF_H0 != 56
constexpr int FRAME_BYTES = B_T33_END;
#endif
constexpr int OUT_FRAME_BYTES = G3 * G3 * 18;
constexpr int IN_FRAME_BYTES = G0 * G0 * 3;

enum { EPI_LUT = 0, EPI_RAW = 1, EPI_ADD = 2, EPI_HEAD = 3, EPI_HEAD_LDS = 4 };

typedef unsigned v4u __attribute__((ext_vector_type(4)));
typedef unsigned v2u __attribute__((ext_vector_type(2)));
typedef unsigned long v4ul __attribute__((ext_vector_type(4)));
template <bool AFTER_MFMA, bool SIGNLESS = false>
__device__ __forceinline__ void rq4(const v4i acc, const v4u m2, const v4u zr, const v4ul c64, int (&t)[4]) {
  v2u d0, d1, d2, d3;
  if constexpr (SIGNLESS) {
    (void)zr;
#define YF_RQ3_MADS "v_mad_u64_u32 %0, vcc, %4, %8, %12\n\tv_mad_u64_u32 %1, vcc, %5, %9, %13\n\t" \
                    "v_mad_u64_u32 %2, vcc, %6, %10, %14\n\tv_mad_u64_u32 %3, vcc, %7, %11, %15"
#define YF_RQ3_OPS : "=&v"(d0), "=&v"(d1), "=&v"(d2), "=&v"(d3) \
                   : "v"(acc[0]), "v"(acc[1]), "v"(acc[2]), "v"(acc[3]), "v"(m2[0]), "v"(m2[1]), "v"(m2[2]), "v"(m2[3]), \
                     "s"(c64[0]), "s"(c64[1]), "s"(c64[2]), "s"(c64[3]) : "vcc"
    if constexpr (AFTER_MFMA) asm("s_nop 7\n\ts_nop 1\n\t" YF_RQ3_MADS YF_RQ3_OPS);
    else asm(YF_RQ3_MADS YF_RQ3_OPS);
#undef YF_RQ3_MADS
#undef YF_RQ3_OPS
    t[0] = (int)d0[1]; t[1] = (int)d1[1]; t[2] = (int)d2[1]; t[3] = (int)d3[1];
    return;
  }
  unsigned long cy0, cy1, cy2, cy3;
#define YF_RQ4_MADS "v_mad_u64_u32 %0, %4, %8, %12, %16\n\tv_mad_u64_u32 %1, %5, %9, %13, %17\n\t" \
                    "v_mad_u64_u32 %2, %6, %10, %14, %18\n\tv_mad_u64_u32 %3, %7, %11, %15, %19"
#define YF_RQ4_OPS : "=&v"(d0), "=&v"(d1), "=&v"(d2), "=&v"(d3), "=&s"(cy0), "=&s"(cy1), "=&s"(cy2), "=&s"(cy3) \
                   : "v"(acc[0]), "v"(acc[1]), "v"(acc[2]), "v"(acc[3]), "v"(m2[0]), "v"(m2[1]), "v"(m2[2]), "v"(m2[3]), \
                     "s"(c64[0]), "s"(c64[1]), "s"(c64[2]), "s"(c64[3])
  if constexpr (AFTER_MFMA) asm("s_nop 7\n\ts_nop 1\n\t" YF_RQ4_MADS YF_RQ4_OPS);
  else asm(YF_RQ4_MADS YF_RQ4_OPS);
#undef YF_RQ4_MADS
#undef YF_RQ4_OPS
  asm("v_addc_co_u32_e64 %0, vcc, %4, %8, %12\n\tv_addc_co_u32_e64 %1, vcc, %5, %9, %13\n\t"
      "v_addc_co_u32_e64 %2, vcc, %6, %10, %14\n\tv_addc_co_u32_e64 %3, vcc, %7, %11, %15"
      : "=&v"(t[0]), "=&v"(t[1]), "=&v"(t[2]), "=&v"(t[3])
      : "v"(zr[0]), "v"(zr[1]), "v"(zr[2]), "v"(zr[3]), "v"(d0[1]), "v"(d1[1]), "v"(d2[1]), "v"(d3[1]),
        "s"(cy0), "s"(cy1), "s"(cy2), "s"(cy3)
      : "vcc");
}
__device__ __forceinline__ int rqf(int acc, uint32_t fs, int k) {
  const float p = (float)acc * __uint_as_float(fs);
  return min(max(__float_as_int(p + 0x1.8p23f) - k, 0), 255);
}
template <bool AFTER_MFMA, bool SIGNLESS = false, bool FP32 = false>
__device__ __forceinline__ void requant4(const v4i acc, const v4u m2, const v4u zr, const v4ul c64, const v4i rs, int (&idx)[4]) {
  if constexpr (FP32) {
    (void)zr; (void)c64;
#pragma unroll
    for (int j = 0; j < 4; ++j) idx[j] = rqf(acc[j], m2[j], rs[j]);
    return;
  }
  int t[4];
  rq4<AFTER_MFMA, SIGNLESS>(acc, m2, zr, c64, t);
#pragma unroll
  for (int j = 0; j < 4; ++j) idx[j] = min(max(t[j] >> rs[j], 0), 255);
}
template <bool AFTER_MFMA, bool SIGNLESS = false, bool FP32 = false>
__device__ __forceinline__ void requant2(const v4i acc, const v4u m2, const v4u zr, const v4ul c64, const v4i rs, int (&idx)[2]) {
  if constexpr (FP32) {
    (void)zr; (void)c64;
    idx[0] = rqf(acc[0], m2[0], rs[0]);
    idx[1] = rqf(acc[1], m2[1], rs[1]);
    return;
  }
  v2u d0, d1;
  if constexpr (SIGNLESS) {
    (void)zr;
    if constexpr (AFTER_MFMA)
      asm("s_nop 7\n\ts_nop 1\n\tv_mad_u64_u32 %0, vcc, %2, %4, %6\n\tv_mad_u64_u32 %1, vcc, %3, %5, %7"
          : "=&v"(d0), "=&v"(d1) : "v"(acc[0]), "v"(acc[1]), "v"(m2[0]), "v"(m2[1]), "s"(c64[0]), "s"(c64[1]) : "vcc");
    else
      asm("v_mad_u64_u32 %0, vcc, %2, %4, %6\n\tv_mad_u64_u32 %1, vcc, %3, %5, %7"
          : "=&v"(d0), "=&v"(d1) : "v"(acc[0]), "v"(acc[1]), "v"(m2[0]), "v"(m2[1]), "s"(c64[0]), "s"(c64[1]) : "vcc");
    idx[0] = min(max((int)d0[1] >> rs[0], 0), 255);
    idx[1] = min(max((int)d1[1] >> rs[1], 0), 255);
    return;
  }
  unsigned long cy0, cy1;
  int t0, t1;
  if constexpr (AFTER_MFMA)
    asm("s_nop 7\n\ts_nop 1\n\tv_mad_u64_u32 %0, %2, %4, %6, %8\n\tv_mad_u64_u32 %1, %3, %5, %7, %9"
        : "=&v"(d0), "=&v"(d1), "=&s"(cy0), "=&s"(cy1) : "v"(acc[0]), "v"(acc[1]), "v"(m2[0]), "v"(m2[1]), "s"(c64[0]), "s"(c64[1]));
  else
    asm("v_mad_u64_u32 %0, %2, %4, %6, %8\n\tv_mad_u64_u32 %1, %3, %5, %7, %9"
        : "=&v"(d0), "=&v"(d1), "=&s"(cy0), "=&s"(cy1) : "v"(acc[0]), "v"(acc[1]), "v"(m2[0]), "v"(m2[1]), "s"(c64[0]), "s"(c64[1]));
  asm("v_addc_co_u32_e64 %0, vcc, %2, %4, %6\n\tv_addc_co_u32_e64 %1, vcc, %3, %5, %7"
      : "=&v"(t0), "=&v"(t1) : "v"(zr[0]), "v"(zr[1]), "v"(d0[1]), "v"(d1[1]), "s"(cy0), "s"(cy1) : "vcc");
  idx[0] = min(max(t0 >> rs[0], 0), 255);
  idx[1] = min(max(t1 >> rs[1], 0), 255);
}
__device__ __forceinline__ uint32_t join2(uint32_t b0, uint32_t b1) {
  uint32_t v;
  asm("v_lshl_or_b32 %0, %1, 8, %2" : "=v"(v) : "v"(b1), "v"(b0));
  return v;
}
constexpr int ACC0 = YF_ACC_OFFSET;
#ifdef YF_RQ3_DENSE
constexpr bool DENSE_SIGNLESS = true;
#else
constexpr bool DENSE_SIGNLESS = false;
#endif
#ifdef YF_RQ_FP32
constexpr bool RQ_FP32 = true;
#else
constexpr bool RQ_FP32 = false;
#endif
__device__ __forceinline__ v4i acc_init(const v4u zr) {
  if constexpr (RQ_FP32) return (v4i)zr;
  else { (void)zr; return v4i{ACC0, ACC0, ACC0, ACC0}; }
}
__device__ __forceinline__ int any_value() { int u; asm volatile("" : "=v"(u)); return u; }
__device__ __forceinline__ int clampi(int v, int lo, int hi) { return min(max(v, lo), hi); }
__device__ __forceinline__ uint32_t join4(uint32_t b0, uint32_t b1, uint32_t b2, uint32_t b3) {
  uint32_t lo, hi, v;
  asm("v_lshl_or_b32 %0, %1, 8, %2" : "=v"(lo) : "v"(b1), "v"(b0));
  asm("v_lshl_or_b32 %0, %1, 8, %2" : "=v"(hi) : "v"(b3), "v"(b2));
  asm("v_lshl_or_b32 %0, %1, 16, %2" : "=v"(v) : "v"(hi), "v"(lo));
  return v;
}
typedef const __attribute__((address_space(3))) uint8_t* lds_u8_ptr;
template <int LUT_ID>
__device__ __forceinline__ uint32_t lutb(int idx) {
  return *(lds_u8_ptr)(uint32_t)(LUT_ID * 256 + idx);
}
__device__ __forceinline__ uint32_t pkmax(uint32_t a, uint32_t b) {
  v2s x, y; __builtin_memcpy(&x, &a, 4); __builtin_memcpy(&y, &b, 4);
  v2s r = __builtin_elementwise_max(x, y);
  uint32_t o; __builtin_memcpy(&o, &r, 4); return o;
}
__device__ __forceinline__ uint32_t pk_shl8(uint32_t d) {
  v2s x; __builtin_memcpy(&x, &d, 4);
  x = x << 8;
  uint32_t o; __builtin_memcpy(&o, &x, 4); return o;
}
struct SplitB {
  uint32_t o, e;
  __device__ __forceinline__ SplitB() : o(0x80008000u), e(0x80008000u) {}
  __device__ __forceinline__ explicit SplitB(uint32_t d) : o(d), e(pk_shl8(d)) {}
  __device__ __forceinline__ SplitB mx(const SplitB& b) const { SplitB r; r.o = pkmax(o, b.o); r.e = pkmax(e, b.e); return r; }
  __device__ __forceinline__ uint32_t merge() const { return __builtin_amdgcn_perm(o, e, 0x07030501u); }
  __device__ __forceinline__ uint32_t b3() const { return o >> 24; }
  __device__ __forceinline__ uint32_t b2() const { return e >> 24; }
  __device__ __forceinline__ uint32_t b1() const { return (o >> 8) & 255u; }
  __device__ __forceinline__ uint32_t b0() const { return (e >> 8) & 255u; }
};
template <int LUT_ID>
__device__ __forceinline__ uint32_t lut4_raw(const SplitB& v) {
  return join4(lutb<LUT_ID>(v.b0()), lutb<LUT_ID>(v.b1()), lutb<LUT_ID>(v.b2()), lutb<LUT_ID>(v.b3()));
}

__device__ __forceinline__ uint32_t lds_u32(const char* p) { return *reinterpret_cast<const uint32_t*>(p); }
typedef const __attribute__((address_space(4))) v4i* cv4i_ptr;
typedef const __attribute__((address_space(4))) uint32_t* cu32_ptr;
typedef const __attribute__((address_space(4))) v4ul* cv4ul_ptr;
struct I4 { int x, y, z, w; };
__device__ __forceinline__ I4 uniform_int4(const void* p) { const v4i v = *(cv4i_ptr)(uintptr_t)p; return I4{v[0], v[1], v[2], v[3]}; }
__device__ __forceinline__ uint32_t uniform_u32(const void* p) { return *(cu32_ptr)(uintptr_t)p; }
struct PassV { v4u m2, zr; };
#ifdef YF_LAB
__device__ __forceinline__ PassV load_pass_v(const uint8_t* pass, int vz) {
  const v4u* p = reinterpret_cast<const v4u*>(pass + vz);
  return PassV{p[0], p[1]};
}
__device__ __forceinline__ v4i load_wfrag(const uint8_t* p, int vz) {
  (void)vz;
  return *reinterpret_cast<const v4i*>(p);
}
#endif
struct PassS { v4ul c64; v4i rs; };
#ifdef YF_LAB
__device__ __forceinline__ PassS load_pass_s(const uint8_t* pass) {
  return PassS{*(cv4ul_ptr)(uintptr_t)(pass + 32), *(cv4i_ptr)(uintptr_t)(pass + 64)};
}
#endif
struct TablePlan { int w_off[YF_N_DENSE], c_off[YF_N_DENSE], g_off[YF_N_DW], lut_off, total;
                   int vb_off[YF_N_CS], vb_bytes[YF_N_CS], sb_off[YF_N_CS]; };
constexpr int PLAN_COUT[YF_N_DENSE] = {8, 4, 18, 6, 36, 6, 18, 24, 8, 40, 8, 40, 8, 24, 40, 32, 18};
constexpr int PLAN_KROW[YF_N_DENSE] = {YF_CONV1_KROW, 16, 16, 32, 16, 48, 16, 48, 32, 16, 48, 16, 48, 16, 48, 48, 32};
constexpr int PLAN_DWC[YF_N_DW] = {8, 18, 36, 24, 40, 40, 40};
constexpr int plan_passes(int cs) { return yf_cs_dense[cs] >= 0 ? (PLAN_COUT[yf_cs_dense[cs]] + 3) / 4 : (PLAN_DWC[yf_cs_dw[cs]] + 3) / 4; }
constexpr int plan_wbytes(int cs) { return yf_cs_dense[cs] >= 0 ? ((PLAN_COUT[yf_cs_dense[cs]] + 3) & ~3) * PLAN_KROW[yf_cs_dense[cs]] : 0; }
constexpr TablePlan make_plan() {
  TablePlan p = {};
  int off = YF_INDEX_RESERVED;
  for (int i = 0; i < YF_N_DENSE; ++i) {
    const int cp = (PLAN_COUT[i] + 3) & ~3;
    off = (off + 15) & ~15; p.w_off[i] = off; off += cp * PLAN_KROW[i];
    off = (off + 15) & ~15; p.c_off[i] = off; off += (cp / 4) * (int)sizeof(yf_pass);
  }
  for (int i = 0; i < YF_N_DW; ++i) { off = (off + 15) & ~15; p.g_off[i] = off; off += ((PLAN_DWC[i] + 3) / 4) * YF_DW_GROUP_BYTES; }
  off = (off + 15) & ~15; p.lut_off = off; off += YF_N_LUT * 256 + YF_ADDLUT_BYTES + YF_DBG_LUT_BYTES;
  for (int cs = 0; cs < YF_N_CS; ++cs) {
    const int bytes = yf_cs_dense[cs] >= 0 ? plan_wbytes(cs) + plan_passes(cs) * (int)sizeof(yf_pass_v) + (yf_cs_add[cs] >= 0 ? 2048 : 0)
                                           : plan_passes(cs) * YF_DWV_GROUP_BYTES;
    off = (off + 15) & ~15; p.vb_off[cs] = off; p.vb_bytes[cs] = (bytes + 15) & ~15; off += p.vb_bytes[cs];
  }
  for (int cs = 0; cs < YF_N_CS; ++cs) { off = (off + 15) & ~15; p.sb_off[cs] = off; off += plan_passes(cs) * (int)sizeof(yf_pass_s); }
  off = (off + 15) & ~15; off += 64;
  p.total = off;
  return p;
}
constexpr TablePlan PLAN = make_plan();
#ifdef YF_LAB
__device__ __forceinline__ yf_dense load_dense(const uint8_t*, int i) {
  yf_dense d = {};
  d.w_off = (uint32_t)PLAN.w_off[i]; d.c_off = (uint32_t)PLAN.c_off[i];
  return d;
}
__device__ __forceinline__ yf_dw load_dw(const uint8_t*, int i) {
  yf_dw d = {};
  d.g_off = (uint32_t)PLAN.g_off[i];
  return d;
}
#endif
__device__ __forceinline__ int load_halo_zp(const uint8_t* tab, int i) {
  return (int)uniform_u32(tab + offsetof(yf_table_index, halo_zp) + 4 * i);
}

template <int JOBS, int NW>
__device__ __forceinline__ void job_range(int wave, int& j0, int& j1) {
  constexpr int BASE = JOBS / NW, REM = JOBS % NW;
  j0 = wave * BASE + min(wave, REM);
  j1 = j0 + BASE + (wave < REM ? 1 : 0);
}

template <class B, bool RING, int F, int NT>
YF_STAGE_FN void fill_halo(char* frames, int zp, int tid) {
  const uint32_t v = (uint32_t)(zp & 255) * 0x01010101u;
  constexpr int DW = B::S / 4;
  constexpr int HR = B::H + B::PT + (RING ? 1 : 0), WR = B::RS;
  constexpr int NPIX = RING ? (2 * WR + 2 * (HR - 2)) : (WR + HR - 1);
  for (int i = tid; i < F * NPIX * DW; i += NT) {
    const int d = i % DW, t = i / DW, k = t % NPIX, f = t / NPIX;
    int r, c;
    if constexpr (RING) {
      if (k < WR) { r = 0; c = k; }
      else if (k < 2 * WR) { r = HR - 1; c = k - WR; }
      else { const int m = k - 2 * WR; r = 1 + (m >> 1); c = (m & 1) ? WR - 1 : 0; }
    } else {
      if (k < WR) { r = 0; c = k; } else { r = 1 + (k - WR); c = 0; }
    }
    *reinterpret_cast<uint32_t*>(frames + f * B::FS + B::OFF + r * B::ROWB + c * B::S + 4 * d) = v;
  }
}

__device__ __forceinline__ uint32_t funnel(uint32_t hi, uint32_t lo, int sh) { return __builtin_amdgcn_alignbit(hi, lo, sh); }
template <int F, int NT>
YF_STAGE_FN void stage_input(char* frames, const int8_t* __restrict__ in, long first_frame, long n_frames,
                                            int zp, int tid) {
  const uint32_t hv = (uint32_t)(zp & 255) * 0x01010101u;
  constexpr int RSW = B_IN::RS, HH = B_IN::H, WQ = B_IN::W / 4;
  constexpr int PER_FRAME = HH * WQ, TOTAL = F * PER_FRAME, ITERS = (TOTAL + NT - 1) / NT;
  for (int i = tid; i < F * (RSW + HH); i += NT) {
    const int f = i / (RSW + HH), k = i - f * (RSW + HH);
    const int idx = k < RSW ? k : (k - RSW + 1) * RSW + 3;
    *reinterpret_cast<uint32_t*>(frames + f * B_IN::FS + B_IN::OFF + idx * 4) = hv;
  }
  const long rest = n_frames - 1 - first_frame;
  const int lastf = __builtin_amdgcn_readfirstlane((int)(rest < (long)(F - 1) ? rest : (long)(F - 1)));
  const int8_t* base = in + first_frame * IN_FRAME_BYTES;
  static_assert(RSW == B_IN::W + 4 && B_IN::S == 4, "dst = OFF + 16 * (r + y + RSW/4 + 1) relies on rows of W + 4 dwords");
  uint32_t ld[ITERS][3];
#pragma unroll
  for (int it = 0; it < ITERS; ++it) {
    const int i = min(tid + it * NT, TOTAL - 1);
    int f = 0;
#pragma unroll
    for (int k = 1; k < F; ++k) f += (i >= k * PER_FRAME) ? 1 : 0;
    const int r = i - f * PER_FRAME;
    const uint32_t* src = reinterpret_cast<const uint32_t*>(base + (uint32_t)(min(f, lastf) * PER_FRAME + r) * 12u);
    ld[it][0] = src[0]; ld[it][1] = src[1]; ld[it][2] = src[2];
  }
#pragma unroll
  for (int it = 0; it < ITERS; ++it) {
    const int i = tid + it * NT;
    if (ITERS * NT == TOTAL || i < TOTAL) {
      int f = 0;
#pragma unroll
      for (int k = 1; k < F; ++k) f += (i >= k * PER_FRAME) ? 1 : 0;
      const int r = i - f * PER_FRAME;
      uint4 px;
      px.x = ld[it][0];
      px.y = funnel(ld[it][1], ld[it][0], 24);
      px.z = funnel(ld[it][2], ld[it][1], 16);
      px.w = ld[it][2] >> 8;
      const int y = (int)((uint32_t)r / (uint32_t)WQ);
      *reinterpret_cast<uint4*>(frames + f * B_IN::FS + B_IN::OFF + (RSW + 4) * 4 + 16 * (r + y)) = px;
    }
  }
}

constexpr int CAM_FRAME_BYTES = 112 * 112 * 2;
__device__ __forceinline__ uint32_t cam_pixel(uint32_t s0, uint32_t s1) {
  const uint32_t r = ((s0 >> 11) & 0x001F001Fu) + ((s1 >> 11) & 0x001F001Fu);
  const uint32_t g = ((s0 >> 5) & 0x003F003Fu) + ((s1 >> 5) & 0x003F003Fu);
  const uint32_t b = (s0 & 0x001F001Fu) + (s1 & 0x001F001Fu);
  const uint32_t rs = r + (r >> 16), gs = g + (g >> 16), bs = b + (b >> 16);
  return (((rs & 0x7Cu) << 1) | ((gs & 0xFCu) << 8) | ((bs & 0x7Cu) << 17)) ^ 0x00808080u;
}
template <int F, int NT>
YF_STAGE_FN void stage_input_cam(char* frames, const uint8_t* __restrict__ cam, long first_frame, long n_frames, int zp, int tid) {
  const uint32_t hv = (uint32_t)(zp & 255) * 0x01010101u;
  constexpr int RSW = B_IN::RS, HH = B_IN::H, WQ = B_IN::W / 4;
  constexpr int PER_FRAME = HH * WQ, TOTAL = F * PER_FRAME;
  for (int i = tid; i < F * (RSW + HH); i += NT) {
    const int f = i / (RSW + HH), k = i - f * (RSW + HH);
    const int idx = k < RSW ? k : (k - RSW + 1) * RSW + 3;
    *reinterpret_cast<uint32_t*>(frames + f * B_IN::FS + B_IN::OFF + idx * 4) = hv;
  }
  const long rest = n_frames - 1 - first_frame;
  const int lastf = __builtin_amdgcn_readfirstlane((int)(rest < (long)(F - 1) ? rest : (long)(F - 1)));
  const uint8_t* base = cam + first_frame * CAM_FRAME_BYTES;
  constexpr int ITERS = (TOTAL + NT - 1) / NT;
  auto item = [&](int i, int& f, int& r, int& y, const uint8_t*& src) {
    f = 0;
#pragma unroll
    for (int k = 1; k < F; ++k) f += (i >= k * PER_FRAME) ? 1 : 0;
    r = i - f * PER_FRAME;
    y = (int)((uint32_t)r / (uint32_t)WQ);
    const int xq = r - y * WQ;
    src = base + (uint32_t)(min(f, lastf) * CAM_FRAME_BYTES + (2 * y) * 224 + 16 * xq);
  };
  auto commit = [&](int f, int r, int y, const uint4& a, const uint4& c) {
    constexpr uint32_t SWAP = 0x02030001u;
    uint4 px;
    px.x = cam_pixel(__builtin_amdgcn_perm(a.x, a.x, SWAP), __builtin_amdgcn_perm(c.x, c.x, SWAP));
    px.y = cam_pixel(__builtin_amdgcn_perm(a.y, a.y, SWAP), __builtin_amdgcn_perm(c.y, c.y, SWAP));
    px.z = cam_pixel(__builtin_amdgcn_perm(a.z, a.z, SWAP), __builtin_amdgcn_perm(c.z, c.z, SWAP));
    px.w = cam_pixel(__builtin_amdgcn_perm(a.w, a.w, SWAP), __builtin_amdgcn_perm(c.w, c.w, SWAP));
    *reinterpret_cast<uint4*>(frames + f * B_IN::FS + B_IN::OFF + (RSW + 4) * 4 + 16 * (r + y)) = px;
  };
#pragma unroll
  for (int it = 0; it < ITERS; it += 2) {
    const int i0 = tid + it * NT, i1 = i0 + NT;
    int f0, r0, y0, f1, r1, y1;
    const uint8_t *s0, *s1;
    item(min(i0, TOTAL - 1), f0, r0, y0, s0);
    item(min(i1, TOTAL - 1), f1, r1, y1, s1);
    const uint4 a0 = *reinterpret_cast<const uint4*>(s0), c0 = *reinterpret_cast<const uint4*>(s0 + 224);
    const uint4 a1 = *reinterpret_cast<const uint4*>(s1), c1 = *reinterpret_cast<const uint4*>(s1 + 224);
    if (i0 < TOTAL) commit(f0, r0, y0, a0, c0);
    if (it + 1 < ITERS && i1 < TOTAL) commit(f1, r1, y1, a1, c1);
  }
}

struct AddK { uint32_t mo2, zro; unsigned long c64o; int rso; };

#ifdef YF_LAB
#include "yf_lab_stages.hip.h"
#endif

template <int NO, int LIM, class LOADC, class STORE>
__device__ __forceinline__ void pool8_sweep(int o0, LOADC loadc, STORE store) {
  constexpr int NR = NO + 3;
  SplitB r[NR];
#pragma unroll
  for (int jj = 0; jj < NR; ++jj) {
    const int j = o0 - 2 + jj;
    r[jj] = SplitB(loadc(clampi(2 * j + 1, 0, LIM))).mx(SplitB(loadc(clampi(2 * j + 2, 0, LIM))));
  }
  SplitB q[NR - 1];
#pragma unroll
  for (int jj = 0; jj < NR - 1; ++jj) q[jj] = r[jj].mx(r[jj + 1]);
#pragma unroll
  for (int n = 0; n < NO; ++n) store(o0 + n, q[n].mx(q[n + 2]));
}
template <int F, int NT>
YF_STAGE_FN void pool8_h(char* frames, int tid) {
  constexpr int NO = 5, OW = B_HB::W, IH = B_T4::H, NCH = (OW + NO - 1) / NO;
  for (int i = tid; i < F * IH * NCH * 5; i += NT) {
    const int cg = i % 5; int t = i / 5;
    const int k = t % NCH; t /= NCH;
    const int y = t % IH; const int f = t / IH;
    char* fbase = frames + f * B_T4::FS;
    const char* row = fbase + B_T4::at(y, 0) + 4 * cg;
    char* dst = fbase + B_HB::OFF + (y * OW) * 20 + 4 * cg;
    pool8_sweep<NO, B_T4::W - 1>(min(k * NO, OW - NO),
                                 [&](int x) { return lds_u32(row + x * B_T4::S); },
                                 [&](int ox, const SplitB& v) { *reinterpret_cast<uint32_t*>(dst + ox * 20) = v.merge(); });
  }
}
template <int F, int NT, bool STASH = false>
YF_STAGE_FN void pool8_v(char* frames, int tid) {
  constexpr int NO = 5, OW = B_HB::W, OH = B_T14::H, NCH = (OH + NO - 1) / NO;
  static_assert(OH >= NO, "column shorter than one sweep");
  for (int i = tid; i < F * OW * NCH * 5; i += NT) {
    const int cg = i % 5; int t = i / 5;
    const int k = t % NCH; t /= NCH;
    const int ox = t % OW; const int f = t / OW;
    char* fbase = frames + f * B_HB::FS;
    const char* col = fbase + B_HB::OFF + ox * 20 + 4 * cg;
    char* dst = fbase + B_T14::OFF + ox * B_T14::S + 4 * cg;
    pool8_sweep<NO, B_HB::H - 1>(min(k * NO, OH - NO),
                                 [&](int r) { return lds_u32(col + r * (OW * 20)); },
                                 [&](int oy, const SplitB& v) {
                                   *reinterpret_cast<uint32_t*>(dst + oy * (OW * B_T14::S)) = lut4_raw<YF_L_Q21>(v);
                                   if constexpr (STASH) *reinterpret_cast<uint32_t*>(dst + oy * (OW * B_T14::S) + YF_T14_CONV_BASE) = v.merge();
                                 });
  }
}

namespace v2 {
constexpr int LUT_B = YF_N_LUT * 256;
constexpr int JT = LUT_B, JT_B = 896;
constexpr int ZERO = JT + JT_B, ZERO_B = 640;
constexpr int SLOT0 = ZERO + ZERO_B, SLOT_B = 2816;
constexpr int slot(int cs) { return SLOT0 + (cs & 1) * SLOT_B; }
struct Lay56 {
  static constexpr int ZERO = v2::ZERO, JT = v2::JT, JT_BYTES = v2::JT_B;
  static constexpr int slot(int cs) { return v2::slot(cs); }
};
constexpr int max_block() { int m = 0; for (int i = 0; i < YF_N_CS; ++i) m = PLAN.vb_bytes[i] > m ? PLAN.vb_bytes[i] : m; return m; }
static_assert(max_block() <= SLOT_B && SLOT0 % 16 == 0 && SLOT_B % 16 == 0, "a constant block fits a ring slot");

typedef const __attribute__((address_space(3))) v4i* lds_v4i_ptr;
typedef const __attribute__((address_space(3))) v4u* lds_v4u_ptr;
typedef const __attribute__((address_space(3))) uint32_t* lds_u32_ptr;
typedef const __attribute__((address_space(3))) v2u* lds_u2_ptr;
__device__ __forceinline__ v4i lds_v4i(uint32_t a) { return *(lds_v4i_ptr)a; }
__device__ __forceinline__ v4u lds_v4u(uint32_t a) { return *(lds_v4u_ptr)a; }

template <int CS, class LAY = Lay56, int BYTES_ = -1>
__device__ __forceinline__ void fetch_consts(const uint8_t* __restrict__ tab, int wave, int lane) {
  constexpr int BYTES = BYTES_ >= 0 ? BYTES_ : PLAN.vb_bytes[CS], NCHUNK = (BYTES + 1023) / 1024;
  if (wave < NCHUNK) {
    asm volatile("" : "+v"(lane));
    const int off = wave * 1024 + lane * 16;
    if (off < BYTES) {
      const uint8_t* src = tab + PLAN.vb_off[CS] + off;
      const uint32_t dst = (uint32_t)(LAY::slot(CS) + wave * 1024);
      uint32_t keep;
      asm volatile("s_mov_b32 %0, m0\n\ts_mov_b32 m0, %2\n\ts_nop 0\n\tglobal_load_lds_dwordx4 %1, off\n\ts_mov_b32 m0, %0"
                   : "=&s"(keep) : "v"(src), "s"(dst) : "memory");
    }
  }
}

template <int W, int SH = (W > 32 ? 20 : 16)> struct DivW {
  static constexpr uint32_t M = ((1u << SH) + W - 1) / W;
  static constexpr bool ok() { for (uint32_t p = 0; p < 2048; ++p) if (((p * M) >> SH) != p / W) return false; return true; }
  static_assert(ok(), "multiply-shift division is exact on [0, 2048)");
  __device__ static __forceinline__ int div(int p) { return (int)(((uint32_t)p * M) >> SH); }
};

template <int EPI, int LUT_ID, int LA, int STASH_LUT = -1>
__device__ __forceinline__ void epilogue2(char* dstpix, const char* addpix, char* headpix, int chq, int hq, const int (&idx)[4], const AddK& ad,
                                          char* stashpix = nullptr) {
  if constexpr (EPI == EPI_LUT) {
    *reinterpret_cast<uint32_t*>(dstpix + chq) = join4(lutb<LUT_ID>(idx[0]), lutb<LUT_ID>(idx[1]), lutb<LUT_ID>(idx[2]), lutb<LUT_ID>(idx[3]));
    if constexpr (STASH_LUT >= 0) {
      if (stashpix) *reinterpret_cast<uint32_t*>(stashpix + chq) =
          join4(*(lds_u8_ptr)(uint32_t)(STASH_LUT + idx[0]), *(lds_u8_ptr)(uint32_t)(STASH_LUT + idx[1]),
                *(lds_u8_ptr)(uint32_t)(STASH_LUT + idx[2]), *(lds_u8_ptr)(uint32_t)(STASH_LUT + idx[3]));
    }
  } else if constexpr (EPI == EPI_RAW) {
    *reinterpret_cast<uint32_t*>(dstpix + chq) = join4(idx[0], idx[1], idx[2], idx[3]) ^ 0x80808080u;
  } else if constexpr (EPI == EPI_ADD) {
    typedef const __attribute__((address_space(3))) int* lds_i32_ptr;
    if (stashpix) *reinterpret_cast<uint32_t*>(stashpix + chq) = join4(idx[0], idx[1], idx[2], idx[3]) ^ 0x80808080u;
    const uint32_t o = lds_u32(addpix + chq) ^ 0x80808080u;
    v4i sum;
#pragma unroll
    for (int j = 0; j < 4; ++j)
      sum[j] = *(lds_i32_ptr)(uint32_t)(LA + 4 * ((o >> (8 * j)) & 255)) + *(lds_i32_ptr)(uint32_t)(LA + 1024 + 4 * idx[j]);
    int r[4];
    requant4<false>(sum, v4u{ad.mo2, ad.mo2, ad.mo2, ad.mo2}, v4u{ad.zro, ad.zro, ad.zro, ad.zro},
                    v4ul{ad.c64o, ad.c64o, ad.c64o, ad.c64o}, v4i{ad.rso, ad.rso, ad.rso, ad.rso}, r);
    *reinterpret_cast<uint32_t*>(dstpix + chq) = join4(r[0], r[1], r[2], r[3]) ^ 0x80808080u;
  } else {
    const uint32_t v = join4(idx[0], idx[1], idx[2], idx[3]) ^ 0x80808080u;
    uint16_t* dst = reinterpret_cast<uint16_t*>(headpix + hq);
    dst[0] = (uint16_t)v;
    if (hq + 2 < 18) dst[1] = (uint16_t)(v >> 16);
  }
}

template <int EPI, int LUT_ID, int LA>
__device__ __forceinline__ void epilogue2_half(char* dstpix, const char* addpix, int chq, const int (&idx)[2], const AddK& ad) {
  static_assert(EPI == EPI_LUT || EPI == EPI_RAW || EPI == EPI_ADD, "half passes: LUT, raw and residual-add epilogues");
  if constexpr (EPI == EPI_LUT) {
    *reinterpret_cast<uint32_t*>(dstpix + chq) = join2(lutb<LUT_ID>(idx[0]), lutb<LUT_ID>(idx[1]));
  } else if constexpr (EPI == EPI_RAW) {
    *reinterpret_cast<uint32_t*>(dstpix + chq) = join2(idx[0], idx[1]) ^ 0x8080u;
  } else {
    typedef const __attribute__((address_space(3))) int* lds_i32_ptr;
    const uint32_t o = lds_u32(addpix + chq) ^ 0x80808080u;
    v4i sum = {0, 0, 0, 0};
#pragma unroll
    for (int j = 0; j < 2; ++j)
      sum[j] = *(lds_i32_ptr)(uint32_t)(LA + 4 * ((o >> (8 * j)) & 255)) + *(lds_i32_ptr)(uint32_t)(LA + 1024 + 4 * idx[j]);
    int r[2];
    requant2<false>(sum, v4u{ad.mo2, ad.mo2, ad.mo2, ad.mo2}, v4u{ad.zro, ad.zro, ad.zro, ad.zro},
                    v4ul{ad.c64o, ad.c64o, ad.c64o, ad.c64o}, v4i{ad.rso, ad.rso, ad.rso, ad.rso}, r);
    *reinterpret_cast<uint32_t*>(dstpix + chq) = join2(r[0], r[1]) ^ 0x8080u;
  }
}
#if !defined(YF_LAB) || !defined(YF_CHUNK_UNROLL)
#undef YF_CHUNK_UNROLL
#define YF_CHUNK_UNROLL 0
#endif
#define YF_HALF_PASS 1

template <int F, int NW, int TPJ, int KS, int BW, class IN, class OUT, int OUT_CH0, int COUT, int EPI, int LUT_ID, class ADDB, int CS,
          int STASH_OFF = -1, int STASH_S = 0, int STASH_LUT = -1, class LAY = Lay56, int LA_ABS = -1>
YF_STAGE_FN void dense2_stage(char* frames, char* out_all, const uint8_t* __restrict__ tab, const AddK ad, int wave, int lane) {
  constexpr int NP = (COUT + 3) / 4, NCH = (NP + TPJ - 1) / TPJ;
  constexpr int P = IN::P, TOT = F * P;
  constexpr bool FRAME_TILES = P <= 64;
  constexpr int MT = FRAME_TILES ? F : (TOT + 63) / 64;
  constexpr int JOBS = NCH * MT, KROW = 16 * KS;
  constexpr int SLOT = LAY::slot(CS), WB = plan_wbytes(CS), PV = SLOT + WB, LA = LA_ABS >= 0 ? LA_ABS : PV + NP * (int)sizeof(yf_pass_v);
  static_assert(yf_cs_dense[CS] >= 0 && KROW == PLAN_KROW[yf_cs_dense[CS]] && NP == plan_passes(CS), "stage and constant block agree");
  static_assert((EPI == EPI_ADD) == (yf_cs_add[CS] >= 0), "residual-add tables travel with their stage");
  static_assert(OUT::P == P || EPI == EPI_HEAD || EPI == EPI_HEAD_LDS, "1x1 conv keeps the grid");
  static_assert(IN::FS == OUT::FS && IN::FS == ADDB::FS, "one frame stride per stage");
  static_assert(IN::S >= 16 * (KS - 1) + BW && (BW == 4 || BW == 8 || BW == 16), "the pixel vector must cover all k-steps");
  static_assert(IN::RS == IN::W && IN::PT == 0 && IN::PL == 0, "dense inputs are plain buffers");
  const int g = lane >> 4, c = lane & 15;
  const bool a_on = (c >> 2) == g;
  const uint32_t a_lane = a_on ? (uint32_t)(SLOT + (c & 3) * KROW) : (uint32_t)LAY::ZERO;
  const uint32_t a_step = a_on ? (uint32_t)(TPJ * 4 * KROW) : 0u;
  const uint8_t* sc = tab + PLAN.sb_off[CS];
  int in_c = 0, out_c = 0, add_c = 0, stash_c = 0;
  static_assert(STASH_OFF < 0 || EPI == EPI_ADD || (EPI == EPI_LUT && STASH_LUT >= 0), "a stash is the pre-add convolution output or a second LUT's view");
  if constexpr (FRAME_TILES) {
    const int p = min(lane, P - 1);
    in_c = IN::OFF + p * IN::S;
    if constexpr (EPI == EPI_HEAD || EPI == EPI_HEAD_LDS) out_c = p * 18;
    else if constexpr (OUT::RS == OUT::W && OUT::PT == 0 && OUT::PL == 0) out_c = OUT::OFF + p * OUT::S + OUT_CH0;
    else { const int y = DivW<OUT::W>::div(p); out_c = OUT::at(y, p - y * OUT::W) + OUT_CH0; }
    add_c = ADDB::OFF + p * ADDB::S;
    if constexpr (STASH_OFF >= 0) stash_c = STASH_OFF + p * STASH_S;
  }
  int j0, j1;
  job_range<JOBS, NW>(wave, j0, j1);
  auto run_chunk = [&](const int chunk, int mt, const int n) __attribute__((always_inline)) {
    v4i a[TPJ][KS];
    PassV pv[TPJ];
    PassS ksr[TPJ];
    const uint32_t a_addr = a_lane + (uint32_t)chunk * a_step;
#pragma unroll
    for (int t = 0; t < TPJ; ++t) {
      const int ps = chunk * TPJ + t;
#pragma unroll
      for (int ks = 0; ks < KS; ++ks) a[t][ks] = lds_v4i(a_addr + (uint32_t)(t * 4 * KROW + 16 * ks));
      pv[t].m2 = lds_v4u((uint32_t)(PV + ps * 32));
      pv[t].zr = lds_v4u((uint32_t)(PV + ps * 32 + 16));
      const uint8_t* s = sc + min(ps, NP - 1) * (int)sizeof(yf_pass_s);
      ksr[t] = PassS{*(cv4ul_ptr)(uintptr_t)s, *(cv4i_ptr)(uintptr_t)(s + 32)};
    }
    const int cq = chunk * TPJ * 4;
    const int out_cc = out_c + cq, add_cc = add_c + cq;
    for (int k = 0; k < n; ++k, ++mt) {
      const char* src; char* dstpix = nullptr; const char* addpix = nullptr; char* headpix = nullptr; char* stashpix = nullptr;
      if constexpr (FRAME_TILES) {
        char* fbase = frames + mt * IN::FS;
        src = fbase + in_c;
        dstpix = fbase + out_cc; addpix = fbase + add_cc;
        if constexpr (STASH_OFF >= 0) stashpix = fbase + stash_c + cq;
        if constexpr (EPI == EPI_HEAD) headpix = out_all + mt * OUT_FRAME_BYTES + out_c;
        if constexpr (EPI == EPI_HEAD_LDS) headpix = fbase + OUT::OFF + out_c;
      } else {
        const int q = min(mt * 64 + lane, TOT - 1);
        int f = 0;
#pragma unroll
        for (int i = 1; i < F; ++i) f += (q >= i * P) ? 1 : 0;
        const int p = q - f * P;
        char* fbase = frames + f * IN::FS;
        src = fbase + IN::OFF + p * IN::S;
        if constexpr (EPI == EPI_HEAD) headpix = out_all + f * OUT_FRAME_BYTES + p * 18;
        else if constexpr (EPI == EPI_HEAD_LDS) headpix = fbase + OUT::OFF + p * 18;
        else if constexpr (OUT::RS == OUT::W && OUT::PT == 0 && OUT::PL == 0) dstpix = fbase + cq + OUT::OFF + p * OUT::S + OUT_CH0;
        else { const int y = DivW<OUT::W>::div(p); dstpix = fbase + cq + OUT::at(y, p - y * OUT::W) + OUT_CH0; }
        if constexpr (EPI == EPI_ADD) addpix = fbase + cq + ADDB::OFF + p * ADDB::S;
        if constexpr (STASH_OFF >= 0) stashpix = fbase + cq + STASH_OFF + p * STASH_S;
      }
      v4i b[KS];
#pragma unroll
      for (int ks = 0; ks < KS - 1; ++ks) b[ks] = *reinterpret_cast<const v4i*>(src + 16 * ks);
      const char* last = src + 16 * (KS - 1);
      if constexpr (BW == 16) b[KS - 1] = *reinterpret_cast<const v4i*>(last);
      else if constexpr (BW == 8) { const int2 t2 = *reinterpret_cast<const int2*>(last); b[KS - 1] = v4i{t2.x, t2.y, any_value(), any_value()}; }
      else b[KS - 1] = v4i{*reinterpret_cast<const int*>(last), any_value(), any_value(), any_value()};
#pragma unroll
      for (int t = 0; t < TPJ; ++t) {
        const int ps = chunk * TPJ + t;
        if (ps < NP) {
          v4i acc = acc_init(pv[t].zr);
#pragma unroll
          for (int ks = 0; ks < KS; ++ks) acc = __builtin_amdgcn_mfma_i32_16x16x64_i8(a[t][ks], b[ks], acc, 0, 0, 0);
          constexpr bool HALF_L = YF_HALF_PASS && COUT % 4 == 2 && STASH_OFF < 0 && (EPI == EPI_LUT || EPI == EPI_RAW || EPI == EPI_ADD);
          const bool half = HALF_L && t == (NP - 1) % TPJ && ps == NP - 1;
          if (half) {
            if constexpr (HALF_L) {
              int idx2[2];
              requant2<true, DENSE_SIGNLESS, RQ_FP32>(acc, pv[t].m2, pv[t].zr, ksr[t].c64, ksr[t].rs, idx2);
              epilogue2_half<EPI, LUT_ID, LA>(dstpix, addpix, t * 4, idx2, ad);
            }
          } else {
            int idx[4];
            requant4<true, DENSE_SIGNLESS, RQ_FP32>(acc, pv[t].m2, pv[t].zr, ksr[t].c64, ksr[t].rs, idx);
            epilogue2<EPI, LUT_ID, LA, STASH_LUT>(dstpix, addpix, headpix, t * 4, ps * 4, idx, ad, stashpix);
          }
        }
      }
    }
  };
  if constexpr (NCH <= YF_CHUNK_UNROLL) {
#pragma unroll
    for (int chunk = 0; chunk < NCH; ++chunk) {
      const int lo = max(j0, chunk * MT), hi = min(j1, (chunk + 1) * MT);
      if (lo < hi) run_chunk(chunk, lo - chunk * MT, hi - lo);
    }
  } else {
    int chunk = (int)((uint32_t)j0 / (uint32_t)MT), mt = j0 - chunk * MT, left = j1 - j0;
    while (left > 0) {
      const int n = min(left, MT - mt);
      run_chunk(chunk, mt, n);
      left -= n; ++chunk; mt = 0;
    }
  }
}

template <int F, int NW, int CS, class IN = B_IN, class OUT = B_T1, class LAY = Lay56>
YF_STAGE_FN void conv1_2_stage(char* frames, const uint8_t* __restrict__ tab, int wave, int lane) {
  constexpr int P = OUT::P, W1 = OUT::W, RSW = IN::RS, TOT = F * P;
  constexpr int MT = (TOT + 63) / 64;
  constexpr int SLOT = LAY::slot(CS), WB = plan_wbytes(CS), PV = SLOT + WB;
  const int g = lane >> 4, c = lane & 15;
  const bool a_on = (c >> 2) == g;
  const uint32_t a_addr = a_on ? (uint32_t)(SLOT + (c & 3) * YF_CONV1_KROW) : (uint32_t)LAY::ZERO;
  const uint8_t* sc = tab + PLAN.sb_off[CS];
  v4i a[2][3];
  PassV pv[2];
#pragma unroll
  for (int ps = 0; ps < 2; ++ps) {
#pragma unroll
    for (int ks = 0; ks < 3; ++ks) a[ps][ks] = lds_v4i(a_addr + (uint32_t)(ps * 4 * YF_CONV1_KROW + 16 * ks));
    pv[ps].m2 = lds_v4u((uint32_t)(PV + ps * 32));
    pv[ps].zr = lds_v4u((uint32_t)(PV + ps * 32 + 16));
  }
  int j0, j1;
  job_range<MT, NW>(wave, j0, j1);
  const AddK ad = {};
  for (int mt = j0; mt < j1; ++mt) {
    const int q = min(mt * 64 + lane, TOT - 1);
    int f = 0;
#pragma unroll
    for (int i = 1; i < F; ++i) f += (q >= i * P) ? 1 : 0;
    const int p = q - f * P;
    const int oy = DivW<W1>::div(p), ox = p - oy * W1;
    char* fbase = frames + f * IN::FS;
    const uint32_t* src = reinterpret_cast<const uint32_t*>(fbase + IN::OFF) + (2 * oy * RSW + 2 * ox + 3);
    const v4i b0 = {(int)src[0], (int)src[1], (int)src[2], (int)src[RSW]};
    const v4i b1 = {(int)src[RSW + 1], (int)src[RSW + 2], (int)src[2 * RSW], (int)src[2 * RSW + 1]};
    const v4i b2 = {(int)src[2 * RSW + 2], any_value(), any_value(), any_value()};
    char* dstpix = fbase + OUT::at(oy, ox);
#pragma unroll
    for (int ps = 0; ps < 2; ++ps) {
      const uint8_t* s = sc + ps * (int)sizeof(yf_pass_s);
      const PassS k = PassS{*(cv4ul_ptr)(uintptr_t)s, *(cv4i_ptr)(uintptr_t)(s + 32)};
      v4i acc = acc_init(pv[ps].zr);
      acc = __builtin_amdgcn_mfma_i32_16x16x64_i8(a[ps][0], b0, acc, 0, 0, 0);
      acc = __builtin_amdgcn_mfma_i32_16x16x64_i8(a[ps][1], b1, acc, 0, 0, 0);
      acc = __builtin_amdgcn_mfma_i32_16x16x64_i8(a[ps][2], b2, acc, 0, 0, 0);
      int idx[4];
      requant4<true, DENSE_SIGNLESS, RQ_FP32>(acc, pv[ps].m2, pv[ps].zr, k.c64, k.rs, idx);
      epilogue2<EPI_LUT, YF_L_LEAKY2, 0>(dstpix, nullptr, nullptr, 4 * ps, 0, idx, ad);
    }
  }
}

struct DwWalk { int R, FG; };
template <int F, int STRIDE, int W, int H>
constexpr DwWalk dw_rows_per_lane() {
#if YF_H0 == 56
  if (STRIDE == 1 && F == 2 && W == 28 && H == 28) return DwWalk{7, 1};
  if (STRIDE == 1 && F == 2 && W == 14 && H == 14) return DwWalk{2, 1};
  if (STRIDE == 2 && F == 2 && W == 14 && H == 14) return DwWalk{7, 2};
  if (STRIDE == 2 && F == 4 && W == 7 && H == 7) return DwWalk{4, 2};
#endif
  return DwWalk{1, 1};
}
template <int F, int STRIDE, class IN, class OUT>
struct DwGeo {
  static constexpr int W = OUT::W, H = OUT::H;
  static constexpr DwWalk WK = dw_rows_per_lane<F, STRIDE, OUT::W, OUT::H>();
  static constexpr int R = WK.R, FG = WK.FG, RG = 4 / FG, BR = RG * R;
  static constexpr int FL = (W <= 8 && F % 2 == 0) ? 2 : 1;
  static constexpr int NSEG = (W + 15) / 16, NRB = (H + BR - 1) / BR, NFP = F / (FL * FG);
  static constexpr int JPG = NFP * NRB * NSEG;
  static_assert(OUT::RS == W && OUT::PT == 0 && OUT::PL == 0, "depthwise outputs are plain buffers");
  static_assert(IN::FS == OUT::FS, "one frame stride per stage");
  static_assert((H >= BR || (R > 1 && H >= R)) && (W >= 16 || W * FL <= 16) && F % (FL * FG) == 0 && RG * FG == 4, "tile shape");
  __device__ static __forceinline__ int seg_row(int rs) { return BR > H ? min(rs * R, H - R) : rs * R; }
  __device__ static __forceinline__ uint2 job(int jj) {
    const int fp = jj / (NRB * NSEG); int rem = jj - fp * (NRB * NSEG);
    const int rb = rem / NSEG, seg = rem - rb * NSEG;
    const int oy0 = BR > H ? 0 : min(rb * BR, H - BR);
    const int x0 = (W >= 16) ? min(seg * 16, W - 16) : 0;
    const int fb = fp * FL * FG * IN::FS;
    return uint2{(uint32_t)(fb + IN::OFF + (oy0 * STRIDE) * IN::ROWB + x0 * STRIDE * IN::S), (uint32_t)(fb + OUT::OFF + (oy0 * W + x0) * OUT::S)};
  }
};
#if YF_H0 == 56
template <int F, bool BATCH>
struct JobTabs {
  typedef TailBufs<BATCH ? FRAME_STRIDE / 2 : FRAME_STRIDE> U;
  static constexpr int FT = BATCH ? 2 * F : F;
  static constexpr int JT_DW3 = 0;
  static constexpr int JT_DW10 = JT_DW3 + 8 * DwGeo<F, 1, B_T1, B_T2>::JPG;
  static constexpr int JT_DW15 = JT_DW10 + 8 * DwGeo<F, 2, B_T4, B_T6>::JPG;
  static constexpr int JT_DW27 = JT_DW15 + 8 * DwGeo<F, 1, B_T8, B_T9>::JPG;
  static constexpr int JT_DW32 = JT_DW27 + 8 * DwGeo<FT, 2, typename U::T15, typename U::T17>::JPG;
  static constexpr int END = JT_DW32 + 8 * DwGeo<FT, 1, typename U::T19, typename U::T20>::JPG;
  static_assert(END <= JT_B, "job tables fit");
};
#endif
template <class B, bool RING, int F>
struct HaloGeo {
  static constexpr int HR = B::H + B::PT + (RING ? 1 : 0), WR = B::RS;
  static constexpr int NPIX = RING ? (2 * WR + 2 * (HR - 2)) : (WR + HR - 1);
  static constexpr int N = F * NPIX;
  static_assert(B::S % 4 == 0 && B::OFF % 4 == 0 && B::FS % 4 == 0, "dword pixels");
  __device__ static __forceinline__ uint32_t entry(int i) {
    const int f = i / NPIX, k = i - f * NPIX;
    int r, c;
    if constexpr (RING) {
      if (k < WR) { r = 0; c = k; }
      else if (k < 2 * WR) { r = HR - 1; c = k - WR; }
      else { const int m = k - 2 * WR; r = 1 + (m >> 1); c = (m & 1) ? WR - 1 : 0; }
    } else {
      if (k < WR) { r = 0; c = k; } else { r = 1 + (k - WR); c = 0; }
    }
    return (uint32_t)(f * B::FS + B::OFF + r * B::ROWB + c * B::S);
  }
};
#if YF_H0 == 56
template <int F, bool BATCH>
struct HaloTabs {
  typedef TailBufs<BATCH ? FRAME_STRIDE / 2 : FRAME_STRIDE> U;
  static constexpr int FT = BATCH ? 2 * F : F;
  typedef HaloGeo<B_T1, true, F> G1; typedef HaloGeo<B_T4, false, F> G4; typedef HaloGeo<B_T8, true, F> G8;
  typedef HaloGeo<B_T15, false, F> G15; typedef HaloGeo<typename U::T19, true, FT> G19;
  static constexpr int H_T1 = 0, H_T4 = H_T1 + 2 * G1::N, H_T8 = H_T4 + 2 * G4::N, H_T15 = H_T8 + 2 * G8::N, H_T19 = H_T15 + 2 * G15::N;
  static constexpr int BYTES = (H_T19 + 2 * G19::N + 15) & ~15;
};
constexpr int HT = SLOT0 + 2 * SLOT_B;
template <int F, bool BATCH> constexpr int pre_bytes() { return HT + HaloTabs<F, BATCH>::BYTES; }
template <class G, int HOFF, int NT>
__device__ __forceinline__ void build_halotab(char* smem, int tid) {
  for (int i = tid; i < G::N; i += NT) *reinterpret_cast<uint16_t*>(smem + HT + HOFF + 2 * i) = (uint16_t)(G::entry(i) >> 2);
}
template <class B, class G, int HOFF>
YF_STAGE_FN void fill_halo_t(char* frames, int zp, int tid) {
  typedef const __attribute__((address_space(3))) uint16_t* lds_u16_ptr;
  if (tid < G::N) {
    const uint32_t v = (uint32_t)(zp & 255) * 0x01010101u;
    char* p = frames + 4u * (uint32_t)*(lds_u16_ptr)(uint32_t)(HT + HOFF + 2 * tid);
    if constexpr (B::S % 8 == 0 && B::OFF % 8 == 0 && B::FS % 8 == 0) {
#pragma unroll
      for (int d = 0; d < B::S / 8; ++d) *reinterpret_cast<uint2*>(p + 8 * d) = uint2{v, v};
    } else {
#pragma unroll
      for (int d = 0; d < B::S / 4; ++d) *reinterpret_cast<uint32_t*>(p + 4 * d) = v;
    }
  }
}
#endif

template <int F, int STRIDE, class IN, class OUT, int JTOFF, class LAY = Lay56>
__device__ __forceinline__ void fill_jobtab(char* smem, int tid) {
  typedef DwGeo<F, STRIDE, IN, OUT> G;
  static_assert(JTOFF % 8 == 0 && JTOFF + G::JPG * 8 <= LAY::JT_BYTES, "job table in bounds");
  if (tid < G::JPG) *reinterpret_cast<uint2*>(smem + LAY::JT + JTOFF + 8 * tid) = G::job(tid);
}

template <int F, int NW, int STRIDE, class IN, class OUT, int C, int LUT_ID, int CS, int JTOFF, class LAY = Lay56>
YF_STAGE_FN void dw2_stage(char* frames, const uint8_t* __restrict__ tab, int wave, int lane) {
  typedef DwGeo<F, STRIDE, IN, OUT> G;
  constexpr int W = G::W, FL = G::FL, JPG = G::JPG;
  constexpr int NG = (C + 3) / 4, JOBS = NG * JPG;
  constexpr int DROW = STRIDE * IN::ROWB;
  constexpr int TS = IN::S, TR = IN::ROWB;
  constexpr int SLOT = LAY::slot(CS);
  static_assert(yf_cs_dw[CS] >= 0 && NG == plan_passes(CS), "stage and constant block agree");
  const int g = lane >> 4, c = lane & 15;
  const int fl = (FL == 2) ? (c >> 3) : 0;
  const int xl = (FL == 2) ? min(c & 7, W - 1) : min(c, W - 1);
  const int fr = fl + FL * (g / G::RG), row0 = G::seg_row(g % G::RG);
  const char* lane_in = frames + fr * IN::FS + row0 * DROW + xl * STRIDE * IN::S;
  char* lane_out = frames + fr * IN::FS + (row0 * W + xl) * OUT::S;
  const bool a_on = (c >> 2) == g;
  const uint32_t a_lane = a_on ? (uint32_t)(SLOT + 4 * (c & 3)) : (uint32_t)LAY::ZERO;
  const uint32_t a_step = a_on ? (uint32_t)YF_DWV_GROUP_BYTES : 0u;
  const uint8_t* sc = tab + PLAN.sb_off[CS];
  int j, j1;
  job_range<JOBS, NW>(wave, j, j1);
  int cg = (int)((uint32_t)j / (uint32_t)JPG), jj = j - cg * JPG, left = j1 - j;
  while (left > 0) {
    const uint32_t wa = a_lane + (uint32_t)cg * a_step;
    v4i a0, a1, a2 = {0, 0, 0, 0};
    a0 = v4i{(int)*(lds_u32_ptr)(wa), (int)*(lds_u32_ptr)(wa + 16), (int)*(lds_u32_ptr)(wa + 32), (int)*(lds_u32_ptr)(wa + 48)};
    a1 = v4i{(int)*(lds_u32_ptr)(wa + 64), (int)*(lds_u32_ptr)(wa + 80), (int)*(lds_u32_ptr)(wa + 96), (int)*(lds_u32_ptr)(wa + 112)};
    a2[0] = (int)*(lds_u32_ptr)(wa + 128);
    PassV pv;
    pv.m2 = lds_v4u((uint32_t)(SLOT + cg * YF_DWV_GROUP_BYTES + 144));
    pv.zr = lds_v4u((uint32_t)(SLOT + cg * YF_DWV_GROUP_BYTES + 160));
    const uint8_t* s = sc + cg * (int)sizeof(yf_pass_s);
    const PassS k = PassS{*(cv4ul_ptr)(uintptr_t)s, *(cv4i_ptr)(uintptr_t)(s + 32)};
    const char* lin = lane_in + 4 * cg;
    char* lout = lane_out + 4 * cg;
    auto entry = [&](int job) { return *(lds_u2_ptr)(uint32_t)(LAY::JT + JTOFF + 8 * min(job, JPG - 1)); };
    auto taps = [&](const v2u e, v4i& b0, v4i& b1, v4i& b2, char*& dst) {
      const char* src = lin + e[0];
      b0[0] = (int)lds_u32(src);               b0[1] = (int)lds_u32(src + TS);          b0[2] = (int)lds_u32(src + 2 * TS);
      b0[3] = (int)lds_u32(src + TR);          b1[0] = (int)lds_u32(src + TR + TS);     b1[1] = (int)lds_u32(src + TR + 2 * TS);
      b1[2] = (int)lds_u32(src + 2 * TR);      b1[3] = (int)lds_u32(src + 2 * TR + TS); b2[0] = (int)lds_u32(src + 2 * TR + 2 * TS);
      dst = lout + e[1];
    };
    auto conv = [&](const v4i& b0, const v4i& b1, const v4i& b2) {
      v4i acc = acc_init(pv.zr);
      acc = __builtin_amdgcn_mfma_i32_16x16x64_i8(a0, b0, acc, 0, 0, 0);
      acc = __builtin_amdgcn_mfma_i32_16x16x64_i8(a1, b1, acc, 0, 0, 0);
      return __builtin_amdgcn_mfma_i32_16x16x64_i8(a2, b2, acc, 0, 0, 0);
    };
    auto finish = [&](const v4i& acc, char* dst) {
      if (YF_HALF_PASS && C % 4 == 2 && cg == NG - 1) {
        int idx2[2];
        requant2<true, false, RQ_FP32>(acc, pv.m2, pv.zr, k.c64, k.rs, idx2);
        *reinterpret_cast<uint32_t*>(dst) = join2(lutb<LUT_ID>(idx2[0]), lutb<LUT_ID>(idx2[1]));
      } else {
        int idx[4];
        requant4<true, false, RQ_FP32>(acc, pv.m2, pv.zr, k.c64, k.rs, idx);
        *reinterpret_cast<uint32_t*>(dst) = join4(lutb<LUT_ID>(idx[0]), lutb<LUT_ID>(idx[1]), lutb<LUT_ID>(idx[2]), lutb<LUT_ID>(idx[3]));
      }
    };
    const int n = min(left, JPG - jj);
    if constexpr (G::R > 1) {
      const v4i ar[3] = {v4i{a0[0], a0[1], a0[2], 0}, v4i{a0[3], a1[0], a1[1], 0}, v4i{a1[2], a1[3], a2[0], 0}};
      for (int i = 0; i < n; ++i) {
        const v2u e = entry(jj + i);
        const char* src = lin + e[0];
        char* dst = lout + e[1];
        auto row = [&](int r) {
          const char* p = src + r * TR;
          return v4i{(int)lds_u32(p), (int)lds_u32(p + TS), (int)lds_u32(p + 2 * TS), any_value()};
        };
        v4i w0 = row(0), w1 = row(1);
#pragma unroll
        for (int y = 0; y < G::R; ++y) {
          if constexpr (STRIDE == 2) { if (y > 0) w1 = row(2 * y + 1); }
          const v4i w2 = row(STRIDE * y + 2);
          v4i acc = acc_init(pv.zr);
          acc = __builtin_amdgcn_mfma_i32_16x16x64_i8(ar[0], w0, acc, 0, 0, 0);
          acc = __builtin_amdgcn_mfma_i32_16x16x64_i8(ar[1], w1, acc, 0, 0, 0);
          acc = __builtin_amdgcn_mfma_i32_16x16x64_i8(ar[2], w2, acc, 0, 0, 0);
          finish(acc, dst + y * W * OUT::S);
          if constexpr (STRIDE == 2) w0 = w2;
          else { w0 = w1; w1 = w2; }
        }
      }
      left -= n; ++cg; jj = 0;
      continue;
    }
    int i = 0;
    v2u e0 = entry(jj), e1 = entry(jj + 1);
    for (; i + 1 < n; i += 2) {
      v4i p0, p1, p2 = {0, any_value(), any_value(), any_value()}, q0, q1, q2 = {0, any_value(), any_value(), any_value()};
      char *dp, *dq;
      taps(e0, p0, p1, p2, dp);
      taps(e1, q0, q1, q2, dq);
      e0 = entry(jj + i + 2); e1 = entry(jj + i + 3);
      const v4i ap = conv(p0, p1, p2);
      const v4i aq = conv(q0, q1, q2);
      finish(ap, dp);
      finish(aq, dq);
    }
    if (i < n) {
      v4i b0, b1, b2 = {0, any_value(), any_value(), any_value()};
      char* dst;
      taps(e0, b0, b1, b2, dst);
      finish(conv(b0, b1, b2), dst);
    }
    left -= n; ++cg; jj = 0;
  }
}
template <int FT> constexpr int pool25_waves() { return (FT * 42 + 63) / 64; }
template <int FT, class T15, class T30, bool STASH = false>
YF_STAGE_FN void pool25_cols(char* frames, int item) {
  static_assert(T15::W == 14 && T15::H == 14 && T30::W == 7 && T15::FS == T30::FS, "pool_25 geometry");
  const int t = DivW<6>::div(item), cg = item - 6 * t;
  const int f = DivW<7>::div(t), ox = t - 7 * f;
  if (f >= FT) return;
  char* fbase = frames + f * T15::FS;
  const char* base = fbase + T15::at(0, 0) + 4 * cg;
  constexpr int S = T15::S, ROW = T15::ROWB;
  const int c0 = max(2 * ox - 1, 0) * S, c1 = 2 * ox * S, c2 = c1 + S, c3 = min(2 * ox + 2, 13) * S;
  auto hrow = [&](int r) {
    const char* p = base + r * ROW;
    return SplitB(lds_u32(p + c0)).mx(SplitB(lds_u32(p + c1))).mx(SplitB(lds_u32(p + c2))).mx(SplitB(lds_u32(p + c3)));
  };
  char* dst = fbase + T30::OFF + ox * T30::S + 4 * cg;
  SplitB prev = hrow(0);
#pragma unroll
  for (int oy = 0; oy < 7; ++oy) {
    SplitB next = hrow(2 * oy + 1);
    if (2 * oy + 2 <= 13) next = next.mx(hrow(2 * oy + 2));
    const SplitB mxv = prev.mx(next);
    *reinterpret_cast<uint32_t*>(dst + oy * (7 * T30::S)) = lut4_raw<YF_L_Q45>(mxv);
    if constexpr (STASH) *reinterpret_cast<uint32_t*>(dst + oy * (7 * T30::S) + 24) = mxv.merge();
    prev = next;
  }
}
}
#ifndef YF_GENERIC
#include "yf_fused56.hip.h"
#else
#ifdef YF_LAB
#include "yf_lab_layerwise.hip.h"
#endif
#include "yf_band160.hip.h"
#endif

}
#pragma clang diagnostic pop
```

Before: 31.61 million images/s.

## Use 32-bit frame indices, scalar-base global loads, and kernarg reloads to cut VGPR/SGPR pressure

Replaces 64-bit long frame and group indices throughout the fused kernel with 32-bit ints, guarded by a host-side check that the frame count fits. Global loads now use scalar base plus 32-bit vector offset addressing (global_load_lds with an saddr operand). Kernel arguments are reread directly from the kernarg segment at each use instead of being held live in registers. The parked-frame state is encoded into a sign bit of the loop counter. The aim is to reduce 64-bit address arithmetic and register pressure, which may help occupancy or scheduling. In exchange it caps launch sizes at 32-bit frame counts and adds fragile inline-asm register-class constraints.

```diff
diff --git a/stm32h7-yolo_amd/csrc/yf_decode.hip.h b/stm32h7-yolo_amd/csrc/yf_decode.hip.h
--- a/stm32h7-yolo_amd/csrc/yf_decode.hip.h
+++ b/stm32h7-yolo_amd/csrc/yf_decode.hip.h
@@ -68,10 +68,11 @@
 }
 
 typedef const __attribute__((address_space(3))) uint32_t* dec_lds_u32;
-__device__ __forceinline__ void decode_frame_lds(const int8_t* head, long frame, int lane, int mode, float w_scale, float h_scale,
+__device__ __forceinline__ void decode_frame_lds(const int8_t* head, int frame, int lane, int mode, float w_scale, float h_scale,
                                                  yf_det* __restrict__ dets, int* __restrict__ counts, int cap, uint32_t lds_tabs, int q_thr) {
-  yf_det* out = dets + frame * cap;
-  const float anc_w[3] = {9.f, 12.f, 22.f}, anc_h[3] = {14.f, 17.f, 21.f};
+  char* out = reinterpret_cast<char*>(dets) + (size_t)(uint32_t)frame * (size_t)(uint32_t)cap * sizeof(yf_det);
+  auto anc_w = [](int a) { return a == 0 ? 9.f : a == 1 ? 12.f : 22.f; };
+  auto anc_h = [](int a) { return a == 0 ? 14.f : a == 1 ? 17.f : 21.f; };
   auto sig = [&](int q) { return __uint_as_float(*(dec_lds_u32)(lds_tabs + 4u * (uint32_t)(q + 128))); };
   auto ex = [&](int q) { return __uint_as_float(*(dec_lds_u32)(lds_tabs + 1024u + 4u * (uint32_t)(q + 128))); };
   int pos[3], off[3], q4[3];
@@ -104,7 +105,7 @@
       d.frame = (int32_t)frame; d.anchor = (uint8_t)a; d.row = (uint8_t)row; d.col = (uint8_t)col;
       d.q_conf = (int8_t)q4[c]; d.conf = sig(q4[c]);
       const float cx = (sx + (float)col) * 8.f, cy = (sy + (float)row) * 8.f;
-      const float bw = ew * anc_w[a], bh = eh * anc_h[a];
+      const float bw = ew * anc_w(a), bh = eh * anc_h(a);
       if (mode == YF_DECODE_PY) {
         float x1 = cx - bw / 2, y1 = cy - bh / 2, x2 = cx + bw / 2, y2 = cy + bh / 2;
         x1 *= w_scale; x2 *= w_scale; y1 *= h_scale; y2 *= h_scale;
@@ -120,10 +121,10 @@
         if (y2 > 55) y2 = 55;
         d.x1 = dbl_wrap(x1); d.y1 = dbl_wrap(y1); d.x2 = dbl_wrap(x2); d.y2 = dbl_wrap(y2);
       }
-      out[pos[c]] = d;
+      *reinterpret_cast<yf_det*>(out + (uint32_t)pos[c] * (uint32_t)sizeof(yf_det)) = d;
     }
   }
-  if (lane == 0) counts[frame] = total;
+  if (lane == 0) counts[(uint32_t)frame] = total;
 }
 
 }
diff --git a/stm32h7-yolo_amd/csrc/yf_engine.hip b/stm32h7-yolo_amd/csrc/yf_engine.hip
--- a/stm32h7-yolo_amd/csrc/yf_engine.hip
+++ b/stm32h7-yolo_amd/csrc/yf_engine.hip
@@ -470,6 +470,8 @@
 
 static const Variant* shape_for(const yf_engine* e, long n) { return (e->var_small && n <= SMALL_N) ? e->var_small : e->var; }
 
+static bool yf_frames_fit_int32(long n, int f, long grid) { return n <= (long)INT32_MAX - 2L * f * grid; }
+
 static int launch(yf_engine* e, const Variant* v, const void* d_in, void* d_out, void* d_dump, long n, hipStream_t s, int stop_stage = -1,
                   const DecodeArgs* dec = nullptr) {
   if (n <= 0) return YF_ENG_OK;
@@ -488,11 +490,12 @@
   if (e->grid_div > 1) grid = grid / e->grid_div > 0 ? grid / e->grid_div : 1;
 #endif
   if (grid > groups) grid = groups;
+  if (!yf_frames_fit_int32(n, v->f, grid)) { e->err = "too many frames for one launch (32-bit frame numbers inside the kernel)"; return YF_ENG_ERR_ARG; }
   prm.scratch = nullptr;
   yf_stream_scratch::Lease lease;
   if (v->park) {
     const size_t need = (size_t)grid * v->f * v->park;
-    if (need > e->park_region) { e->err = "tail scratch region too small for this kernel shape"; return YF_ENG_ERR_VARIANT; }
+    if (need > e->park_region || need > 0xffffffffu) { e->err = "tail scratch region too small for this kernel shape"; return YF_ENG_ERR_VARIANT; }
     HIPCHK(e, e->park.get(s, e->park_region, &lease));
     prm.scratch = lease.ptr;
   }
diff --git a/stm32h7-yolo_amd/csrc/yf_fused56.hip.h b/stm32h7-yolo_amd/csrc/yf_fused56.hip.h
--- a/stm32h7-yolo_amd/csrc/yf_fused56.hip.h
+++ b/stm32h7-yolo_amd/csrc/yf_fused56.hip.h
@@ -49,6 +49,13 @@
   char* scratch;
 };
 static_assert(sizeof(yf_table_index) <= YF_INDEX_RESERVED, "index does not fit its reserved slot");
+typedef const __attribute__((address_space(4))) char* kargs_ptr;
+__device__ __forceinline__ kargs_ptr kargs_here() {
+  kargs_ptr p = (kargs_ptr)__builtin_amdgcn_kernarg_segment_ptr();
+  asm volatile("" : "+s"(p));
+  return p;
+}
+#define YF_ARG(FIELD) (*reinterpret_cast<const __attribute__((address_space(4))) decltype(NetParams::FIELD)*>(kargs_here() + offsetof(NetParams, FIELD)))
 
 #ifndef YF_POOL_MERGE
 #define YF_POOL_MERGE 1
@@ -98,20 +105,23 @@
   constexpr int FT = BATCH ? 2 * F : F;
   typedef TailBufs<BATCH ? FRAME_STRIDE / 2 : FRAME_STRIDE> U;
   constexpr int OUT_ALL_BYTES = BATCH ? 0 : (F * OUT_FRAME_BYTES + 15) & ~15;
+  static_assert(std::is_same<decltype(&yoloface56_fused<F, NW, DUMP, CAM>), void (*)(const NetParams)>::value, "YF_ARG: NetParams is the kernel's only argument (kernarg offset 0)");
   uint8_t* luts = reinterpret_cast<uint8_t*>(smem);
   constexpr int PRE = v2::pre_bytes<F, tail_batch<DUMP>()>();
   char* out_all = smem + PRE;
   char* frames = smem + PRE + OUT_ALL_BYTES;
-  long parked_first = -1;
+  const int n_frames = (int)prm.n;
   const int tid0 = threadIdx.x;
   const uint8_t* __restrict__ tab = prm.tab;
   int vz = 0;
   asm volatile("" : "+v"(vz));
+  const __attribute__((address_space(1))) uint8_t* lut_src = (const __attribute__((address_space(1))) uint8_t*)(tab + PLAN.lut_off);
+  asm volatile("" : "+s"(lut_src));
   for (int i = tid0; i < v2::LUT_B / 16; i += NT)
-    reinterpret_cast<uint4*>(luts)[i] = reinterpret_cast<const uint4*>(tab + PLAN.lut_off)[i];
+    reinterpret_cast<v4u*>(luts)[i] = *(const __attribute__((address_space(1))) v4u*)(lut_src + (uint32_t)(16 * i));
   for (int i = tid0; i < v2::ZERO_B / 16; i += NT) reinterpret_cast<uint4*>(smem + v2::ZERO)[i] = uint4{0, 0, 0, 0};
   constexpr int DBG_LUT = PRE + OUT_ALL_BYTES + FRAME_BYTES + (F - 1) * FRAME_STRIDE;
-  if constexpr (DUMP) { if (tid0 < YF_DBG_LUT_BYTES / 16) reinterpret_cast<uint4*>(smem + DBG_LUT)[tid0] = reinterpret_cast<const uint4*>(tab + PLAN.lut_off + YF_N_LUT * 256 + YF_ADDLUT_BYTES)[tid0]; }
+  if constexpr (DUMP) { if (tid0 < YF_DBG_LUT_BYTES / 16) reinterpret_cast<v4u*>(smem + DBG_LUT)[tid0] = *(const __attribute__((address_space(1))) v4u*)(lut_src + (uint32_t)(YF_N_LUT * 256 + YF_ADDLUT_BYTES + 16 * tid0)); }
 #if !(defined(YF_LAB) && defined(YF_WHATIF_NO_PROLOGUE_TABLES))
   {
     typedef v2::JobTabs<F, tail_batch<DUMP>()> JTS;
@@ -130,7 +140,11 @@
   }
 #endif
 
-  const long n_groups = (prm.n + F - 1) / F;
+  auto sfresh = [](int v) { asm volatile("" : "+s"(v)); return v; };
+  auto n_groups = [&]() { return (int)((uint32_t)(sfresh(n_frames) + F - 1) / (uint32_t)F); };
+  int gstep = (int)gridDim.x;
+  asm volatile("" : "+s"(gstep));
+  auto park_slot = [&]() { return YF_ARG(scratch) + (uint32_t)(sfresh((int)blockIdx.x) * (F * TailBufs<FRAME_BYTES>::T15_BYTES)); };
   const AddK no_add = {};
   auto addctx = [&](int k) {
     const uint8_t* a = tab + offsetof(yf_table_index, add) + k * sizeof(yf_add);
@@ -150,32 +164,35 @@
 #define YF_SYNC() do { asm volatile("s_waitcnt vmcnt(0)" ::: "memory"); __syncthreads(); } while (0)
 #endif
 #define YF_HALO(B, RING, FR, G, HOFF, WI, TID) \
-  v2::fill_halo_t<B, typename v2::HaloTabs<F, BATCH>::G, v2::HaloTabs<F, BATCH>::HOFF>(frames, load_halo_zp(tab, WI), TID)
-#define YF_FETCH(CS, WV, LN) v2::fetch_consts<CS>(tab, WV, LN)
+  do { int ht_ = TID; asm volatile("" : "+v"(ht_)); \
+       v2::fill_halo_t<B, typename v2::HaloTabs<F, BATCH>::G, v2::HaloTabs<F, BATCH>::HOFF>(frames, load_halo_zp(tab, WI), ht_); } while (0)
+#define YF_FETCH(CS, WV, LN) v2::fetch_consts_s<CS>(tab, WV, LN)
 #define YF_CONV1(WV, LN, CS) v2::conv1_2_stage<F, NW, CS>(frames, tab, WV, LN)
 #define YF_DENSE(FR, TPJ, KS, BW, IN, OUT, CH0, COUT, EPI, LUT, ADDB, DI, AD, WV, LN, CS) \
   v2::dense2_stage<FR, NW, TPJ, KS, BW, IN, OUT, CH0, COUT, EPI, LUT, ADDB, CS>(frames, out_all, tab, AD, WV, LN)
 #define YF_DW(FR, STRIDE, IN, OUT, C, LUT, WI, WV, LN, CS, JTOFF) v2::dw2_stage<FR, NW, STRIDE, IN, OUT, C, LUT, CS, v2::JobTabs<F, BATCH>::JTOFF>(frames, tab, WV, LN)
 #define YF_DUMP(BUF, C, OFF, ...) \
-  if constexpr (DUMP) { if (prm.dump) { dump_buf<BUF, C, F, NT>(frames, prm.dump, DS, DumpOffsets::OFF, first, prm.n, tid, ##__VA_ARGS__); YF_SYNC(); } }
+  if constexpr (DUMP) { if (prm.dump) { dump_buf<BUF, C, F, NT>(frames, prm.dump, DS, DumpOffsets::OFF, first, n_frames, tid, ##__VA_ARGS__); YF_SYNC(); } }
   int stage_no = 0;
 #define YF_STAGE_END() if constexpr (DUMP) { if (++stage_no == prm.stop_stage) continue; }
 #define YF_PRIO(K) stage_prio<K>()
 
-  long prev_first = -1;
+  int prev_first = -1;
   auto decode_prev = [&](int w, int ln) {
-    if (prm.dets != nullptr && prev_first >= 0 && w >= NW - F && prev_first + (w - (NW - F)) < prm.n) {
+    if (prm.dets != nullptr && prev_first >= 0 && w >= NW - F && prev_first + (w - (NW - F)) < n_frames) {
       int dl = ln;
       asm volatile("" : "+v"(dl));
       yfdec::decode_frame(reinterpret_cast<const int8_t*>(out_all) + (w - (NW - F)) * OUT_FRAME_BYTES, prev_first + (w - (NW - F)), dl,
                           prm.mode, prm.w_scale, prm.h_scale, prm.dets, prm.counts, prm.cap);
     }
   };
-  for (long grp = blockIdx.x; grp < n_groups; grp += gridDim.x) {
-    const long first = grp * F;
+  constexpr int PARKED = (int)0x80000000;
+  for (int st = blockIdx.x; (st & ~PARKED) < n_groups(); st += gstep) {
+    const int grp = st & ~PARKED;
+    const int first = grp * F;
 #ifdef YF_BARPROF
     bar_no = 0;
-    prof_on = !DUMP && prm.dump != nullptr && grp == (long)blockIdx.x + gridDim.x;
+    prof_on = !DUMP && prm.dump != nullptr && grp == (int)blockIdx.x + gstep;
 #endif
     int tid = tid0, tid_f = tid0, tid_m = tid0, tid_t = tid0;
     if constexpr ((YF_LAUNDER & 1) != 0) asm volatile("" : "+v"(tid_f));
@@ -195,8 +212,8 @@
     YF_PRIO(0);
     int tid_s = tid0;
     asm volatile("" : "+v"(tid_s));
-    if constexpr (CAM) stage_input_cam<F, NT>(frames, reinterpret_cast<const uint8_t*>(prm.in), first, prm.n, (int)uniform_u32(tab + offsetof(yf_table_index, in_zp)), tid_s);
-    else stage_input<F, NT>(frames, prm.in, first, prm.n, (int)uniform_u32(tab + offsetof(yf_table_index, in_zp)), tid_s);
+    if constexpr (CAM) stage_input_cam<F, NT>(frames, reinterpret_cast<const uint8_t*>(YF_ARG(in)), first, n_frames, (int)uniform_u32(tab + offsetof(yf_table_index, in_zp)), tid_s);
+    else stage_input<F, NT>(frames, YF_ARG(in), first, n_frames, (int)uniform_u32(tab + offsetof(yf_table_index, in_zp)), tid_s);
     YF_FETCH(0, W_f, L_f);
     YF_HALO(B_T1, true, F, G1, H_T1, YF_W_DW3, tid_f);
     YF_SYNC();
@@ -286,13 +303,13 @@
     YF_STAGE_END()
     YF_PRIO(13);
     if constexpr (BATCH) {
-      if (parked_first >= 0) {
+      if (st < 0) {
         constexpr int PV = TailBufs<FRAME_BYTES>::T15_BYTES / 16, WI = (PV + 63) / 64;
-        const char* park = prm.scratch + (long)blockIdx.x * (F * PV * 16);
+        const char* park = park_slot();
         for (int j = W_m; j < F * WI; j += NW) {
           const int f = j / WI, k0 = (j - f * WI) * 64;
           if (k0 + L_m < PV)
-            __builtin_amdgcn_global_load_lds((const __attribute__((address_space(1))) void*)(uintptr_t)(park + (f * PV + k0 + L_m) * 16),
+            __builtin_amdgcn_global_load_lds((const __attribute__((address_space(1))) void*)(uintptr_t)(park + (uint32_t)((f * PV + k0 + L_m) * 16)),
                                              (__attribute__((address_space(3))) void*)(uintptr_t)(uint32_t)(PRE + (2 * f + 1) * U::T15::FS + 16 * k0),
                                              16, 0, 0);
         }
@@ -304,31 +321,34 @@
     if constexpr (BATCH) asm volatile("s_waitcnt vmcnt(0)" ::: "memory");
     YF_SYNC(); YF_DUMP(B_T15, 24, T15)
     YF_STAGE_END()
-    long odd_first = -1;
+    int odd_first = -1;
     if constexpr (BATCH) {
       constexpr int V = U::T15_BYTES / 16;
-      uint4* park = reinterpret_cast<uint4*>(prm.scratch) + (long)blockIdx.x * (F * V);
-      if (parked_first < 0 && grp + gridDim.x < n_groups) {
+      static_assert(U::T15_BYTES == TailBufs<FRAME_BYTES>::T15_BYTES, "one slot size for the park stores and the DMA back");
+      if (st >= 0 && grp + gstep < n_groups()) {
+        char* park = park_slot();
+        __builtin_assume(tid_t >= 0 && tid_t < NT);
         for (int i = tid_t; i < F * V; i += NT) {
           const int f = i / V, k = i - f * V;
-          park[i] = *reinterpret_cast<const uint4*>(frames + f * FRAME_STRIDE + 16 * k);
+          *reinterpret_cast<uint4*>(park + (uint32_t)(16 * i)) = *reinterpret_cast<const uint4*>(frames + f * FRAME_STRIDE + 16 * k);
         }
-        parked_first = first;
+        st |= PARKED;
         continue;
       }
-      if (parked_first >= 0) {
-        odd_first = parked_first;
-        parked_first = -1;
+      if (st < 0) {
+        odd_first = (grp - gstep) * F;
+        st &= ~PARKED;
       }
     }
-    auto frame_of = [&](int f) -> long {
-      long id = first + f;
-      if constexpr (BATCH) id = (f & 1) ? (odd_first >= 0 ? odd_first + (f >> 1) : -1) : first + (f >> 1);
-      return id < prm.n ? id : -1;
+    const int first_t = sfresh(grp) * F;
+    auto frame_of = [&](int f) -> int {
+      int id = first_t + f;
+      if constexpr (BATCH) id = (f & 1) ? (odd_first >= 0 ? odd_first + (f >> 1) : -1) : first_t + (f >> 1);
+      return id < n_frames ? id : -1;
     };
 #define YF_DUMP_T(BUF, C, OFF, ...) \
   if constexpr (DUMP) { if (prm.dump) { if constexpr (BATCH) dump_sets<BUF, C, FT, NT>(frames, prm.dump, DS, DumpOffsets::OFF, frame_of, tid, ##__VA_ARGS__); \
-                                        else dump_buf<BUF, C, FT, NT>(frames, prm.dump, DS, DumpOffsets::OFF, first, prm.n, tid, ##__VA_ARGS__); \
+                                        else dump_buf<BUF, C, FT, NT>(frames, prm.dump, DS, DumpOffsets::OFF, first, n_frames, tid, ##__VA_ARGS__); \
                                         YF_SYNC(); } }
     YF_PRIO(14);
     YF_FETCH(12, W_t, L_t);
@@ -405,14 +425,15 @@
     YF_STAGE_END()
     YF_PRIO(25);
     YF_FETCH(23, W_t, L_t);
-    if (BATCH && prm.dets != nullptr && W_t < 2) {
+    if (BATCH && YF_ARG(dets) != nullptr && W_t < 2) {
       int dl = L_t;
       asm volatile("" : "+v"(dl));
-      const uint8_t* src = reinterpret_cast<const uint8_t*>(W_t == 0 ? yfdec::d_sig_bits : yfdec::d_exp_bits) + 16 * dl;
+      const uint8_t* src = reinterpret_cast<const uint8_t*>(sfresh(W_t) == 0 ? yfdec::d_sig_bits : yfdec::d_exp_bits);
+      const uint32_t voff = 16u * (uint32_t)dl;
       const uint32_t dst = (uint32_t)(PRE + OUT_ALL_BYTES + 1024 * W_t);
       uint32_t keep;
-      asm volatile("s_mov_b32 %0, m0\n\ts_mov_b32 m0, %2\n\ts_nop 0\n\tglobal_load_lds_dwordx4 %1, off\n\ts_mov_b32 m0, %0"
-                   : "=&s"(keep) : "v"(src), "s"(dst) : "memory");
+      asm volatile("s_mov_b32 %0, m0\n\ts_mov_b32 m0, %3\n\ts_nop 0\n\tglobal_load_lds_dwordx4 %1, %2\n\ts_mov_b32 m0, %0"
+                   : "=&s"(keep) : "v"(voff), "s"(src), "s"(dst) : "memory");
     }
     YF_DENSE(FT, 2, 3, 16, typename U::T20, typename U::T33, 0, 32, EPI_LUT, YF_L_LEAKY52, typename U::T33, YF_D_C51, no_add, W_t, L_t, 22);
     YF_SYNC(); YF_DUMP_T(typename U::T33, 32, T33)
@@ -421,32 +442,40 @@
     if constexpr (!BATCH) {
       YF_DENSE(FT, 1, 2, 16, typename U::T33, typename U::T33, 0, 18, EPI_HEAD, 0, typename U::T33, YF_D_C53, no_add, W_t, L_t, 23);
       YF_SYNC();
-      const long valid = min((long)F, prm.n - first);
-      const int n16 = (int)(valid * (OUT_FRAME_BYTES / 2));
-      uint16_t* dst = reinterpret_cast<uint16_t*>(prm.out + first * OUT_FRAME_BYTES);
+      const int n16 = min(F, n_frames - first) * (OUT_FRAME_BYTES / 2);
+      int8_t* dst = YF_ARG(out) + (size_t)(uint32_t)first * OUT_FRAME_BYTES;
       const uint16_t* srcp = reinterpret_cast<const uint16_t*>(out_all);
-      for (int i = tid; i < n16; i += NT) dst[i] = srcp[i];
+      for (int i = tid; i < n16; i += NT) *reinterpret_cast<uint16_t*>(dst + (uint32_t)(2 * i)) = srcp[i];
       prev_first = first;
     } else {
       YF_DENSE(FT, 1, 2, 16, typename U::T33, typename U::HEAD, 0, 18, EPI_HEAD_LDS, 0, typename U::T33, YF_D_C53, no_add, W_t, L_t, 23);
       YF_SYNC();
       constexpr int H16 = OUT_FRAME_BYTES / 2;
-      const bool split = prm.dets != nullptr && FT < NW;
+      yf_det* const dets = YF_ARG(dets);
+      int8_t* const heads = YF_ARG(out);
+      const bool split = dets != nullptr && FT < NW;
       const int c0 = split ? tid_t - FT * 64 : tid_t, cstep = split ? NT - FT * 64 : NT;
       if (!split || W_t >= FT) {
-        for (int i = c0; i < FT * H16; i += cstep) {
-          const int f = i / H16, k = i - f * H16;
-          const long id = frame_of(f);
-          if (id >= 0) reinterpret_cast<uint16_t*>(prm.out + id * OUT_FRAME_BYTES)[k] = *reinterpret_cast<const uint16_t*>(frames + f * U::HEAD::FS + U::HEAD::OFF + 2 * k);
+#pragma unroll
+        for (int f = 0; f < FT; ++f) {
+          const int id = frame_of(f);
+          if (id >= 0) {
+            int8_t* dst = heads + (size_t)(uint32_t)id * OUT_FRAME_BYTES;
+            for (int k = c0; k < H16; k += cstep)
+              *reinterpret_cast<uint16_t*>(dst + (uint32_t)(2 * k)) = *reinterpret_cast<const uint16_t*>(frames + f * U::HEAD::FS + U::HEAD::OFF + 2 * k);
+          }
         }
       }
       for (int f = W_t; f < FT; f += NW) {
-        const long id = frame_of(f);
-        if (prm.dets != nullptr && id >= 0) {
+        const int id = frame_of(f);
+        if (dets != nullptr && id >= 0) {
           int dl = L_t;
           asm volatile("" : "+v"(dl));
-          yfdec::decode_frame_lds(reinterpret_cast<const int8_t*>(frames + f * U::HEAD::FS + U::HEAD::OFF), id, dl, prm.mode, prm.w_scale, prm.h_scale, prm.dets, prm.counts, prm.cap,
-                                  (uint32_t)(PRE + OUT_ALL_BYTES), prm.q_thr);
+          const kargs_ptr ka = kargs_here();
+#define YF_ARG_AT(FIELD) (*reinterpret_cast<const __attribute__((address_space(4))) decltype(NetParams::FIELD)*>(ka + offsetof(NetParams, FIELD)))
+          yfdec::decode_frame_lds(reinterpret_cast<const int8_t*>(frames + f * U::HEAD::FS + U::HEAD::OFF), id, dl, YF_ARG_AT(mode), YF_ARG_AT(w_scale), YF_ARG_AT(h_scale), dets,
+                                  YF_ARG_AT(counts), YF_ARG_AT(cap), (uint32_t)(PRE + OUT_ALL_BYTES), YF_ARG_AT(q_thr));
+#undef YF_ARG_AT
         }
       }
     }
@@ -456,6 +485,7 @@
     const int tid = tid0, lane = tid & 63, wave = __builtin_amdgcn_readfirstlane(tid >> 6);
     decode_prev(wave, lane);
   }
+#undef YF_ARG
 #undef YF_HALO
 #undef YF_FETCH
 #undef YF_CONV1
diff --git a/stm32h7-yolo_amd/csrc/yf_kernels.hip.h b/stm32h7-yolo_amd/csrc/yf_kernels.hip.h
--- a/stm32h7-yolo_amd/csrc/yf_kernels.hip.h
+++ b/stm32h7-yolo_amd/csrc/yf_kernels.hip.h
@@ -378,7 +378,7 @@
 
 __device__ __forceinline__ uint32_t funnel(uint32_t hi, uint32_t lo, int sh) { return __builtin_amdgcn_alignbit(hi, lo, sh); }
 template <int F, int NT>
-YF_STAGE_FN void stage_input(char* frames, const int8_t* __restrict__ in, long first_frame, long n_frames,
+YF_STAGE_FN void stage_input(char* frames, const int8_t* __restrict__ in, int first_frame, int n_frames,
                                             int zp, int tid) {
   const uint32_t hv = (uint32_t)(zp & 255) * 0x01010101u;
   constexpr int RSW = B_IN::RS, HH = B_IN::H, WQ = B_IN::W / 4;
@@ -388,9 +388,8 @@
     const int idx = k < RSW ? k : (k - RSW + 1) * RSW + 3;
     *reinterpret_cast<uint32_t*>(frames + f * B_IN::FS + B_IN::OFF + idx * 4) = hv;
   }
-  const long rest = n_frames - 1 - first_frame;
-  const int lastf = __builtin_amdgcn_readfirstlane((int)(rest < (long)(F - 1) ? rest : (long)(F - 1)));
-  const int8_t* base = in + first_frame * IN_FRAME_BYTES;
+  const int lastf = min(n_frames - 1 - first_frame, F - 1);
+  const int8_t* base = in + (size_t)(uint32_t)first_frame * IN_FRAME_BYTES;
   static_assert(RSW == B_IN::W + 4 && B_IN::S == 4, "dst = OFF + 16 * (r + y + RSW/4 + 1) relies on rows of W + 4 dwords");
   uint32_t ld[ITERS][3];
 #pragma unroll
@@ -431,7 +430,7 @@
   return (((rs & 0x7Cu) << 1) | ((gs & 0xFCu) << 8) | ((bs & 0x7Cu) << 17)) ^ 0x00808080u;
 }
 template <int F, int NT>
-YF_STAGE_FN void stage_input_cam(char* frames, const uint8_t* __restrict__ cam, long first_frame, long n_frames, int zp, int tid) {
+YF_STAGE_FN void stage_input_cam(char* frames, const uint8_t* __restrict__ cam, int first_frame, int n_frames, int zp, int tid) {
   const uint32_t hv = (uint32_t)(zp & 255) * 0x01010101u;
   constexpr int RSW = B_IN::RS, HH = B_IN::H, WQ = B_IN::W / 4;
   constexpr int PER_FRAME = HH * WQ, TOTAL = F * PER_FRAME;
@@ -440,9 +439,8 @@
     const int idx = k < RSW ? k : (k - RSW + 1) * RSW + 3;
     *reinterpret_cast<uint32_t*>(frames + f * B_IN::FS + B_IN::OFF + idx * 4) = hv;
   }
-  const long rest = n_frames - 1 - first_frame;
-  const int lastf = __builtin_amdgcn_readfirstlane((int)(rest < (long)(F - 1) ? rest : (long)(F - 1)));
-  const uint8_t* base = cam + first_frame * CAM_FRAME_BYTES;
+  const int lastf = min(n_frames - 1 - first_frame, F - 1);
+  const uint8_t* base = cam + (size_t)(uint32_t)first_frame * CAM_FRAME_BYTES;
   constexpr int ITERS = (TOTAL + NT - 1) / NT;
   auto item = [&](int i, int& f, int& r, int& y, const uint8_t*& src) {
     f = 0;
@@ -500,6 +498,7 @@
 template <int F, int NT>
 YF_STAGE_FN void pool8_h(char* frames, int tid) {
   constexpr int NO = 5, OW = B_HB::W, IH = B_T4::H, NCH = (OW + NO - 1) / NO;
+  __builtin_assume(tid >= 0 && tid < NT);
   for (int i = tid; i < F * IH * NCH * 5; i += NT) {
     const int cg = i % 5; int t = i / 5;
     const int k = t % NCH; t /= NCH;
@@ -516,6 +515,7 @@
 YF_STAGE_FN void pool8_v(char* frames, int tid) {
   constexpr int NO = 5, OW = B_HB::W, OH = B_T14::H, NCH = (OH + NO - 1) / NO;
   static_assert(OH >= NO, "column shorter than one sweep");
+  __builtin_assume(tid >= 0 && tid < NT);
   for (int i = tid; i < F * OW * NCH * 5; i += NT) {
     const int cg = i % 5; int t = i / 5;
     const int k = t % NCH; t /= NCH;
@@ -564,6 +564,22 @@
       uint32_t keep;
       asm volatile("s_mov_b32 %0, m0\n\ts_mov_b32 m0, %2\n\ts_nop 0\n\tglobal_load_lds_dwordx4 %1, off\n\ts_mov_b32 m0, %0"
                    : "=&s"(keep) : "v"(src), "s"(dst) : "memory");
+    }
+  }
+}
+template <int CS>
+__device__ __forceinline__ void fetch_consts_s(const uint8_t* __restrict__ tab, int wave, int lane) {
+  constexpr int BYTES = PLAN.vb_bytes[CS], NCHUNK = (BYTES + 1023) / 1024;
+  asm volatile("" : "+s"(wave));
+  if (wave < NCHUNK) {
+    asm volatile("" : "+v"(lane));
+    const int off = wave * 1024 + lane * 16;
+    if (off < BYTES) {
+      const uint32_t voff = (uint32_t)(PLAN.vb_off[CS] + off);
+      const uint32_t dst = (uint32_t)(Lay56::slot(CS) + wave * 1024);
+      uint32_t keep;
+      asm volatile("s_mov_b32 %0, m0\n\ts_mov_b32 m0, %3\n\ts_nop 0\n\tglobal_load_lds_dwordx4 %1, %2\n\ts_mov_b32 m0, %0"
+                   : "=&s"(keep) : "v"(voff), "s"(tab), "s"(dst) : "memory");
     }
   }
 }
```

Result: faster. 32.15 million images/s (median of 6 runs) (+1.7%).
